# dacase/rnamotif

Measured on NVIDIA B200. Metric: strand-nt scanned per second (both strands), higher is better.
Workload: dtype u8

## Files before the change

rnamotif_b200/csrc/gm_kernel.cuh:

```cuda
#pragma once

#include <cuda_runtime.h>
#include <stdint.h>
#include "gm_search.cuh"
#include "gm_score.h"
#include "gm_twobit.h"
#include "gm_inflate.h"

namespace gm {


#define GM_REC_CACHE 30

#define PV (*L.P)

struct ScanArgs {
	DevParams par;
	const gm_plan_t *plan;
	const DevSearch *ds;
	const uint8_t *packed;
	int64_t total_nt;
	const int64_t *rec_off;
	int n_rec;
	int64_t g_begin, g_end;
// ... 42 lines not shown
			for (int k = 0; k < 4; k++) {
				uint32_t x = 0;
				for (int b = 0; b < 4; b++) {
					int64_t j = i + k * 4 + b;
					x |= (uint32_t)(j < n ? chars[j] : 0) << (8 * b);
				}
				w[k] = x;
			}
		}
		uint32_t out[2] = {0, 0};
		for (int k = 0; k < 16; k++) {
			unsigned ch = (w[k >> 2] >> (8 * (k & 3))) & 0xff;
			unsigned c = ch ? code_of_char(ch) : 0;
			out[k >> 3] |= c << (4 * (k & 7));
		}
		*reinterpret_cast<uint2 *>(packed + (i >> 1)) = make_uint2(out[0], out[1]);
	}
}

__device__ __forceinline__ int64_t last_le(const int64_t *__restrict__ a, int64_t lo, int64_t hi, int64_t x)
{
	while (lo < hi) {
		const int64_t mid = (lo + hi + 1) >> 1;
		if (a[mid] <= x)
			lo = mid;
		else
			hi = mid - 1;
	}
	return lo;
}

__device__ __forceinline__ int64_t first_ge2(const int64_t *__restrict__ a, int64_t lo, int64_t hi, int64_t x)
{
	while (lo < hi) {
		const int64_t mid = (lo + hi) >> 1;
		if (a[2 * mid] < x)
			lo = mid + 1;
		else
			hi = mid;
	}
	return lo;
}

__global__ void __launch_bounds__(256) gm_unpack2_kernel(const uint8_t *__restrict__ src,
	const int64_t *__restrict__ dna_off, const int64_t *__restrict__ rec_off, int n_rec,
	const int64_t *__restrict__ nblk, int64_t n_nblk, int64_t g0, int64_t n, uint8_t *__restrict__ packed)
{
	__shared__ int64_t br[4];
	const int64_t span = 256 * 16, end = g0 + n;
	for (int64_t b0 = g0 + (int64_t)blockIdx.x * span; b0 < end; b0 += (int64_t)gridDim.x * span) {
		const int64_t b1 = min(b0 + span, end);
		if (threadIdx.x == 0)
			br[0] = last_le(rec_off, 0, n_rec - 1, b0);
		else if (threadIdx.x == 1)
			br[1] = last_le(rec_off, 0, n_rec - 1, b1 - 1);
		else if (threadIdx.x == 2) {
			int64_t lo = 0, hi = n_nblk;
			while (lo < hi) {
				const int64_t mid = (lo + hi) >> 1;
				if (nblk[2 * mid + 1] <= b0)
					lo = mid + 1;
				else
					hi = mid;
			}
			br[2] = lo;
		} else if (threadIdx.x == 3)
			br[3] = first_ge2(nblk, 0, n_nblk, b1);
		__syncthreads();
		const int64_t r_lo = br[0], r_hi = br[1], k_lo = br[2], k_hi = br[3];
		const int64_t gg = b0 + (int64_t)threadIdx.x * 16;
		if (gg < b1) {
			const int64_t r = last_le(rec_off, r_lo, r_hi, gg);
			bool fast = gg + 16 <= rec_off[r + 1] && gg + 16 <= end;
			if (fast && k_lo < k_hi) {
				const int64_t k = first_ge2(nblk, k_lo, k_hi, gg + 16) - 1;
				fast = k < k_lo || nblk[2 * k + 1] <= gg;
			}
			uint32_t lo = 0, hi = 0;
			if (fast) {
				const int64_t q = gg - rec_off[r];
				const int phase = (int)(q & 3);
				const uint8_t *s = src + dna_off[r] + (q >> 2);
				const uint32_t be4 = ((uint32_t)s[0] << 24) | ((uint32_t)s[1] << 16) | ((uint32_t)s[2] << 8) | s[3];
				const uint32_t b4 = phase ? s[4] : 0;
				twobit_expand16(twobit_window(be4, b4, phase), lo, hi);
			} else {
				for (int j = 0; j < 16; j++) {
					const int64_t g = gg + j;
					if (g >= end)
						break;
					const int64_t rr = last_le(rec_off, r_lo, r_hi, g);
					const int64_t q = g - rec_off[rr];
					uint32_t code = twobit_code4((src[dna_off[rr] + (q >> 2)] >> (6 - 2 * (int)(q & 3))) & 3);
					if (k_lo < k_hi) {
						const int64_t k = first_ge2(nblk, k_lo, k_hi, g + 1) - 1;
						if (k >= k_lo && g < nblk[2 * k + 1])
							code = 15;
					}
					if (j < 8)
						lo |= code << (4 * j);
					else
						hi |= code << (4 * (j - 8));
				}
			}
			*reinterpret_cast<uint2 *>(packed + (gg >> 1)) = make_uint2(lo, hi);
		}
		__syncthreads();
	}
}

struct BgzfMember {
	uint64_t src;
	uint64_t dst;
	uint32_t len;
	uint32_t isize;
	uint32_t crc;
	uint32_t pad_;
};

__global__ void __launch_bounds__(32) gm_inflate_kernel(const uint8_t *__restrict__ gz, const BgzfMember *__restrict__ mem,
	int m0, int m1, uint8_t *__restrict__ text, uint8_t *__restrict__ status, unsigned int *__restrict__ first_bad)
{
	__shared__ uint32_t crc_tab[256];
	for (int i = threadIdx.x; i < 256; i += blockDim.x)
		crc_tab[i] = crc32_entry((uint32_t)i);
	__syncthreads();
	const int m = m0 + (int)(blockIdx.x * blockDim.x + threadIdx.x);
	if (m >= m1)
		return;
	const BgzfMember e = mem[m];
	uint32_t n_out;
	int st = inflate(gz + e.src, e.len, text + e.dst, e.isize, &n_out);
	if (st == GM_INF_OK && crc32(crc_tab, text + e.dst, e.isize) != e.crc)
		st = GM_INF_CRC;
	status[m] = (uint8_t)st;
	if (st != GM_INF_OK)
		atomicMin(first_bad, (unsigned int)m);
}


__device__ __forceinline__ uint32_t smem_u32(const void *p)
{
	return (uint32_t)__cvta_generic_to_shared(p);
}
__device__ __forceinline__ void mbar_init(uint64_t *bar, int count)
{
	asm volatile("mbarrier.init.shared::cta.b64 [%0], %1;" ::"r"(smem_u32(bar)), "r"(count));
	asm volatile("fence.mbarrier_init.release.cluster;" ::: "memory");
}
__device__ __forceinline__ void mbar_expect_tx(uint64_t *bar, uint32_t bytes)
{
	asm volatile("mbarrier.arrive.expect_tx.shared::cta.b64 _, [%0], %1;" ::"r"(smem_u32(bar)), "r"(bytes)
		: "memory");
}
__device__ __forceinline__ void tma_bulk_g2s(void *dst, const void *src, uint32_t bytes, uint64_t *bar)
{
	asm volatile(
		"cp.async.bulk.shared::cluster.global.mbarrier::complete_tx::bytes [%0], [%1], %2, [%3];" ::"r"(
			smem_u32(dst)),
		"l"(src), "r"(bytes), "r"(smem_u32(bar))
		: "memory");
}
__device__ __forceinline__ void mbar_wait(uint64_t *bar, uint32_t parity)
{
	asm volatile(
		"{\n"
		".reg .pred p;\n"
		"WAIT_%=:\n"
		"mbarrier.try_wait.parity.shared::cta.b64 p, [%0], %1;\n"
		"@p bra DONE_%=;\n"
		"bra WAIT_%=;\n"
		"DONE_%=:\n"
		"}\n" ::"r"(smem_u32(bar)),
		"r"(parity)
		: "memory");
}


__host__ __device__ inline size_t plan_smem_bytes(const DevParams &par)
{
	size_t n = 0;
	n += (sizeof(PlanView) + 15) & ~(size_t)15;
	n += (par.n_searches * sizeof(DevSearch) + 15) & ~(size_t)15;
	n += (par.n_descr * sizeof(gm_elem_t) + 15) & ~(size_t)15;
	n += (par.n_pairsets * sizeof(gm_pairset_t) + 15) & ~(size_t)15;
	n += (par.n_regex * sizeof(DevRegex) + 15) & ~(size_t)15;
	n += ((size_t)par.n_scopes * 4 + 15) & ~(size_t)15;
	n += ((size_t)par.n_lentab + 15) & ~(size_t)15;
	n += (par.n_sites * sizeof(gm_site_t) + 15) & ~(size_t)15;
	n += ((size_t)par.n_descr * 4 + 15) & ~(size_t)15;
	n += 2 * (((size_t)(par.n_descr + 1) * 4 + 15) & ~(size_t)15);
	return n;
}

struct StagedPlan {
	PlanView *pv;
	DevSearch *ds;
	const gm_pairset_t *ps;
	uint32_t *elmm;
	int *pmin, *pmax;
};

__device__ __forceinline__ void copy_words(void *dst, const void *src, int n_words, int tid, int nt)
{
	for (int i = tid; i < n_words; i += nt)
		reinterpret_cast<uint32_t *>(dst)[i] = reinterpret_cast<const uint32_t *>(src)[i];
}

__device__ __forceinline__ uint8_t *stage_plan(uint8_t *p, const ScanArgs &A, int tid, int nt, StagedPlan &sp)
{
	const DevParams &par = A.par;
	const gm_plan_t *pl = A.plan;
	PlanView *pv = reinterpret_cast<PlanView *>(p);         p += (sizeof(PlanView) + 15) & ~(size_t)15;
	DevSearch *ds = reinterpret_cast<DevSearch *>(p);       p += (par.n_searches * sizeof(DevSearch) + 15) & ~(size_t)15;
	gm_elem_t *el = reinterpret_cast<gm_elem_t *>(p);       p += (par.n_descr * sizeof(gm_elem_t) + 15) & ~(size_t)15;
	gm_pairset_t *ps = reinterpret_cast<gm_pairset_t *>(p); p += (par.n_pairsets * sizeof(gm_pairset_t) + 15) & ~(size_t)15;
	DevRegex *rx = reinterpret_cast<DevRegex *>(p);         p += (par.n_regex * sizeof(DevRegex) + 15) & ~(size_t)15;
	int32_t *sc = reinterpret_cast<int32_t *>(p);           p += ((size_t)par.n_scopes * 4 + 15) & ~(size_t)15;
	uint8_t *lt = p;                                        p += ((size_t)par.n_lentab + 15) & ~(size_t)15;
	gm_site_t *si = reinterpret_cast<gm_site_t *>(p);       p += (par.n_sites * sizeof(gm_site_t) + 15) & ~(size_t)15;
	uint32_t *elmm = reinterpret_cast<uint32_t *>(p);       p += ((size_t)par.n_descr * 4 + 15) & ~(size_t)15;
	int *pmin = reinterpret_cast<int *>(p);                 p += ((size_t)(par.n_descr + 1) * 4 + 15) & ~(size_t)15;
	int *pmax = reinterpret_cast<int *>(p);                 p += ((size_t)(par.n_descr + 1) * 4 + 15) & ~(size_t)15;
	for (int i = tid; i < (int)(sizeof(DevParams) / 4); i += nt)
		reinterpret_cast<uint32_t *>(&pv->par)[i] = reinterpret_cast<const uint32_t *>(&A.par)[i];
	copy_words(ds, A.ds, par.n_searches * (int)(sizeof(DevSearch) / 4), tid, nt);
	copy_words(el, pl->elems, par.n_descr * (int)(sizeof(gm_elem_t) / 4), tid, nt);
	copy_words(ps, pl->pairsets, par.n_pairsets * (int)(sizeof(gm_pairset_t) / 4), tid, nt);
	for (int r = 0; r < par.n_regex; r++)
		copy_words(rx + r, &pl->regex[r], (int)(sizeof(DevRegex) / 4), tid, nt);
	copy_words(sc, pl->scopes, par.n_scopes, tid, nt);
	copy_words(lt, pl->lentab, (par.n_lentab + 3) / 4, tid, nt);
	copy_words(si, pl->sites, par.n_sites * (int)(sizeof(gm_site_t) / 4), tid, nt);
	for (int i = tid; i < par.n_descr; i += nt)
		elmm[i] = pk16(pl->elems[i].minlen, pl->elems[i].maxlen);
	if (tid == 0) {
		int a = 0, b = 0;
		for (int i = 0; i <= par.n_descr; i++) {
			pmin[i] = a;
			pmax[i] = b;
			if (i < par.n_descr) {
				a += pl->elems[i].minlen;
				b += pl->elems[i].maxlen;
			}
		}
		pv->elems = el;
		pv->pairsets = ps;
		pv->regex = rx;
		pv->scopes = sc;
		pv->lentab = lt;
		pv->sites = si;
		pv->lctx = pl->lctx;
		pv->rctx = pl->rctx;
		pv->n_sites = par.n_sites;
		pv->n_pairsets = par.n_pairsets;
		pv->n_regex = par.n_regex;
		pv->pad_ = 0;
	}
	sp.pv = pv;
	sp.ds = ds;
	sp.ps = ps;
	sp.elmm = elmm;
	sp.pmin = pmin;
	sp.pmax = pmax;
	return p;
}


__device__ __noinline__ uint32_t el_word_lite(const Lane &L, int d)
{
	const int s = PV.par.elsrc[d];
	const int type = PV.elems[d].type;
	const int z = lo16(L_ZD(L, s));
	if (type == GM_SS)
		return pk16(z, lo16(L_FR(L, s, 0)) - z + 1);
	const int hl = hi16(L_FR(L, s, 3));
	if (type == GM_H5)
		return pk16(z, hl);
	return pk16(hi16(L_FR(L, s, 2)) - hl + 1, hl);
}
__device__ __forceinline__ int m_off(const Lane &L, int d) { return lo16(el_word(L, d, PV.par.lite != 0)); }
__device__ __forceinline__ int m_len(const Lane &L, int d) { return hi16(el_word(L, d, PV.par.lite != 0)); }

__device__ __noinline__ int wtype(const Lane &L, int p)
{
	for (int d = 0; d < L.ND; d++) {
		uint32_t w = el_word(L, d, PV.par.lite != 0);
		int off = lo16(w), len = hi16(w);
		if (len > 0 && p >= off && p < off + len)
			return PV.elems[d].type;
	}
	return -1;
}
__device__ __forceinline__ bool is_ss(const Lane &L, int p, bool undef_is_ss)
{
	int t = wtype(L, p);
	return t == GM_SS || (undef_is_ss && t < 0);
}

__device__ __noinline__ bool sink_strict(const Lane &L)
{
	for (int d = 0; d < L.ND; d++) {
		const gm_elem_t &e = PV.elems[d];
		if (!e.strict)
			continue;
		if (e.type == GM_H5) {
// ... 485 lines not shown
```

rnamotif_b200/csrc/gm_machine.cuh:

```cuda
#pragma once

#include "gm_kernel.cuh"
#include "gm_tilebits.h"

namespace gm {

enum {
	CL_IDLE = 0, CL_SPAN = 1, CL_WX = 2, CL_PK = 3, CL_TR = 4, CL_QU = 5
};
enum {
	PHX_IDLE = 0,
	PHX_ENTER = CL_SPAN * 8, PHX_SPAN, PHX_SS_RESUME, PHX_PH_RESUME, PHX_WC_RESUME,
	PHX_WX_BEGIN = CL_WX * 8, PHX_WX_RESUME, PHX_WX_FIRST, PHX_WX_EXT,
	PHX_PK_S5 = CL_PK * 8, PHX_PK_S3, PHX_PK_SD,
	PHX_TR_RESUME = CL_TR * 8, PHX_TR_S,
	PHX_QU_S1 = CL_QU * 8, PHX_QU_RESUME, PHX_QU_S2
};

#define PH_IDLE PHX_IDLE
#define PH_ENTER PHX_ENTER
#define PH_SPAN PHX_SPAN
#define PH_SS_RESUME PHX_SS_RESUME
#define PH_PH_RESUME PHX_PH_RESUME
#define PH_WC_RESUME PHX_WC_RESUME
#define PH_WX_BEGIN PHX_WX_BEGIN
#define PH_WX_RESUME PHX_WX_RESUME
#define PH_WX_FIRST PHX_WX_FIRST
#define PH_WX_EXT PHX_WX_EXT
#define PH_PK_S5 PHX_PK_S5
#define PH_PK_S3 PHX_PK_S3
#define PH_PK_SD PHX_PK_SD
#define PH_TR_RESUME PHX_TR_RESUME
#define PH_TR_S PHX_TR_S
#define PH_QU_S1 PHX_QU_S1
#define PH_QU_RESUME PHX_QU_RESUME
#define PH_QU_S2 PHX_QU_S2

#define GM_RETURN()                                  \
	do {                                             \
		if (s == 0)                                  \
			ph = PH_IDLE;                            \
		else {                                       \
			s--;                                     \
			ph = hi16(L_FR(L, s, 1));                \
		}                                            \
	} while (0)

#define FR1_LO(mpr, lbpr, chk) (((mpr) & 0xff) | ((lbpr) << 8) | ((chk) << 9))

#define GM_QCAP 128
#define GM_REFILL_MIN 16

struct WarpTile {
	uint64_t bar;
	int r_lo;
	int one_rec;
};

__device__ __forceinline__ uint8_t expand_code(unsigned c)
{
	unsigned b = c == 1 ? 0 : c == 2 ? 1 : c == 4 ? 2 : c == 8 ? 3 : 4;
	return (uint8_t)(c | (b << 4));
}
__device__ __forceinline__ uint8_t complement_byte(uint8_t v)
{
	unsigned b = v >> 4;
	if (b > 3)
		return (uint8_t)(15 | (4 << 4));
	unsigned nb = 3 - b;
	return (uint8_t)((1u << nb) | (nb << 4));
}

__device__ __forceinline__ uint64_t bits64(const uint32_t *set_, int q)
{
	const uint32_t *set = gm_sh(set_);
	const int w = q >> 5, sh = q & 31;
	const uint32_t a = set[w], b = set[w + 1], c = set[w + 2];
	const uint32_t lo = __funnelshift_r(a, b, sh);
	const uint32_t hi = __funnelshift_r(b, c, sh);
	return (uint64_t)lo | ((uint64_t)hi << 32);
}

struct PairBits {
	const uint32_t *base;
	int nwb;
	int n_dups;
};

__device__ __forceinline__ uint64_t wc_mask_body(const PairBits &pb, const uint8_t *sq, int strand, int sqbase,
	int dupi, int flt, int z, int lo, int n)
{
	const uint64_t ones = n >= 64 ? ~0ull : ((1ull << n) - 1);
	const int req = flt & 0xff, budget = (flt >> 8) & 0xff, first_must = (flt >> 16) & 1;
	if (dupi < 0 || req == 0)
		return ones;
	const uint32_t *sets = pb.base + ((size_t)(strand * pb.n_dups + dupi) * 4) * pb.nwb;
	if (budget == 0 && first_must) {
		uint64_t a = ones;
		for (int k = 0; k < req; k++) {
			const int x = bcode_of(sq[z + k]);
			if (x >= 4)
				return 0;
			a &= bits64(sets + x * pb.nwb, sqbase + lo - k);
		}
		return a;
	}
	uint64_t a0 = ones, a1 = ones, a2 = ones;
	for (int k = 0; k < req; k++) {
		const int x = bcode_of(sq[z + k]);
		uint64_t m = 0;
		if (x < 4)
			m = bits64(sets + x * pb.nwb, sqbase + lo - k);
		if (k == 0 && first_must) {
			a0 = a1 = a2 = m;
		} else if (k == 0 && budget == 0) {
		} else {
			a2 = (a2 & m) | a1;
			a1 = (a1 & m) | a0;
			a0 &= m;
		}
	}
	return (budget == 0 ? a0 : budget == 1 ? a1 : a2) & ones;
}

__device__ __noinline__ uint64_t wc_mask(const PairBits &pb, const uint8_t *sq, int strand, int sqbase,
	int dupi, int flt, int z, int lo, int n)
{
	return wc_mask_body(pb, sq, strand, sqbase, dupi, flt, z, lo, n);
}

template <int REQ, typename Fin>
__device__ __forceinline__ uint32_t sieve_word_r(const PairBits &pb, int strand, int dupi, int flt, int w, int Dlo, int Dhi, Fin fin)
{
	constexpr int NS_ = REQ > 0 ? REQ : 8;
	const int req = REQ > 0 ? REQ : (flt & 0xff);
	const int budget = (flt >> 8) & 0xff, first_must = (flt >> 16) & 1;
	const int nwb = pb.nwb;
	const uint32_t *P = gm_sh(pb.base) + ((size_t)(strand * pb.n_dups + dupi) * 4) * nwb;
	const uint32_t *I = gm_sh(pb.base) + ((size_t)(strand * pb.n_dups) * 4) * nwb;
	uint32_t Bl[4], Bh[4];
#pragma unroll
	for (int x = 0; x < 4; x++) {
		Bl[x] = I[x * nwb + w];
		Bh[x] = I[x * nwb + w + 1];
	}
	uint32_t res = 0;
	const int Dmin = Dlo - 2 * (req - 1);
	for (int par = 0; par < 2; par++) {
		uint32_t a0[NS_], a1[NS_];
#pragma unroll
		for (int u = 0; u < NS_; u++)
			a0[u] = a1[u] = ~0u;
		for (int d = Dmin + par; d <= Dhi; d += 2) {
			const int ww = min(w + (d >> 5), nwb - 3), sh = d & 31;
			uint32_t Ml = 0, Mh = 0;
#pragma unroll
			for (int x = 0; x < 4; x++) {
				const uint32_t c0 = P[x * nwb + ww], c1 = P[x * nwb + ww + 1], c2 = P[x * nwb + ww + 2];
				Ml |= Bl[x] & __funnelshift_r(c0, c1, sh);
				Mh |= Bh[x] & __funnelshift_r(c1, c2, sh);
			}
#pragma unroll
			for (int k = NS_ - 1; k >= 1; k--) {
				if (REQ > 0 || k < req) {
					const uint32_t t = __funnelshift_r(Ml, Mh, k);
					a1[k] = (a1[k] & t) | a0[k];
					a0[k] &= t;
				}
			}
			uint32_t f;
			if (first_must)
				f = (budget ? a1[0] : a0[0]) & Ml;
			else if (budget == 0)
				f = a0[0];
			else
				f = (a1[0] & Ml) | a0[0];
			if (d >= Dlo)
				res |= fin(d, f);
#pragma unroll
			for (int u = 0; u < NS_ - 1; u++) {
				a0[u] = a0[u + 1];
				a1[u] = a1[u + 1];
			}
			a0[NS_ - 1] = a1[NS_ - 1] = ~0u;
		}
	}
	return res;
}

template <typename Fin>
__device__ __forceinline__ uint32_t sieve_word(const PairBits &pb, int strand, int dupi, int flt, int w, int Dlo, int Dhi, Fin fin)
{
	return sieve_word_r<0>(pb, strand, dupi, flt, w, Dlo, Dhi, fin);
}
template <typename Fin>
__device__ __forceinline__ uint32_t sieve_word_main(const PairBits &pb, int strand, int dupi, int flt, int w, int Dlo, int Dhi, Fin fin)
{
	switch (flt & 0xff) {
	case 3: return sieve_word_r<3>(pb, strand, dupi, flt, w, Dlo, Dhi, fin);
	case 4: return sieve_word_r<4>(pb, strand, dupi, flt, w, Dlo, Dhi, fin);
	case 5: return sieve_word_r<5>(pb, strand, dupi, flt, w, Dlo, Dhi, fin);
	case 6: return sieve_word_r<6>(pb, strand, dupi, flt, w, Dlo, Dhi, fin);
	case 7: return sieve_word_r<7>(pb, strand, dupi, flt, w, Dlo, Dhi, fin);
	}
	return sieve_word_r<0>(pb, strand, dupi, flt, w, Dlo, Dhi, fin);
}

__device__ __forceinline__ uint32_t bits32(const uint32_t *set_, int q)
{
	const uint32_t *set = gm_sh(set_);
	return __funnelshift_r(set[q >> 5], set[(q >> 5) + 1], q & 31);
}

__device__ __noinline__ uint64_t wc_mask_rev(const PairBits &pb, const uint8_t *sq, int strand, int sqbase,
	int dupi_t, int flt, int e, int zlo, int n)
{
	const uint64_t ones = n >= 64 ? ~0ull : ((1ull << n) - 1);
	const int req = flt & 0xff, budget = (flt >> 8) & 0xff, first_must = (flt >> 16) & 1;
	if (dupi_t < 0 || req == 0)
		return ones;
	const uint32_t *sets = pb.base + ((size_t)(strand * pb.n_dups + dupi_t) * 4) * pb.nwb;
	uint64_t a0 = ones, a1 = ones, a2 = ones;
	for (int k = 0; k < req; k++) {
		const int y = bcode_of(sq[e - k]);
		uint64_t m = 0;
		if (y < 4)
			m = bits64(sets + y * pb.nwb, sqbase + zlo + k);
		if (k == 0 && first_must) {
			a0 = a1 = a2 = m;
		} else if (k == 0 && budget == 0) {
		} else {
			a2 = (a2 & m) | a1;
			a1 = (a1 & m) | a0;
			a0 &= m;
		}
	}
	return (budget == 0 ? a0 : budget == 1 ? a1 : a2) & ones;
}

__device__ __forceinline__ bool tail_feasible(const PairBits &pb, const uint8_t *sq, int strand, int sqbase,
	const DevSearch &S, const DevSearch &T, int s5, int s3, int hl)
{
	const int e = s3 - hl - S.lk_off;
	int zhi = e - T.dlo;
	const int zlo = max(e - T.dhi, s5 + hl);
	for (; zhi >= zlo; zhi -= 64) {
		const int l0 = max(zlo, zhi - 63);
		if (wc_mask_rev(pb, sq, strand, sqbase, T.dupi_t, T.flt, e, l0, zhi - l0 + 1) != 0)
			return true;
	}
	return false;
}

#define GM_LOOK_FWD(any, T, zt, bound)                                   \
	do {                                                                 \
		int f_ = min((bound), (zt) + (T).dhi);                           \
		const int l_ = (zt) + (T).dlo;                                   \
		(any) = false;                                                   \
		for (; f_ >= l_ && !(any); f_ -= 64) {                           \
			const int l0_ = max(l_, f_ - 63);                            \
			(any) = GM_MASK((T), (zt), l0_, f_ - l0_ + 1) != 0;          \
		}                                                                \
	} while (0)

__device__ __noinline__ bool probes_ok(const Lane &L, const DevSearch &S, int s5, int s3, int hl, int wend)
{
	for (int i = 0; i < S.n_probe; i++) {
		const unsigned pr = S.probe[i];
		const int anchor = pr & 3, off = (pr >> 2) & 1023, len = (pr >> 12) & 255;
		const int rxi = (pr >> 20) & 31, mm = (pr >> 25) & 15;
		const int pos = anchor == 0 ? s5 + hl + off : anchor == 1 ? s3 + 1 + off : s3 - hl + 1 - off - len;
		if (pos < 0 || pos + len - 1 > wend)
			return false;
		const DevRegex &rx = PV.regex[rxi];
		int n_mm;
		if (mm > 0 ? !rx_match_mm(rx, L.sq + pos, len, mm, &n_mm) : !rx_match(rx, L.sq + pos, len))
			return false;
	}
	return true;
}

template <int MODE, bool FULL, int PF>
__device__ __forceinline__ void gm_search_body(const ScanArgs &A)
{
	constexpr bool SIEVE = PF >= 2;
	const bool LIT = PF == 1 || (SIEVE && A.par.lit_present != 0);
	extern __shared__ __align__(16) uint8_t smem_raw[];
	const int tid = threadIdx.x, nt = blockDim.x;
	const int lane = tid & 31, warp = tid >> 5;
	const int NS = A.par.n_searches, ND = A.par.n_descr;
	const int W = A.par.w_winsize, H = A.par.halo, TILE = A.par.tile;
	const int Lbytes = (TILE + 2 * H + 31) & ~31;
	const int stage_bytes = ((Lbytes >> 1) + 32 + 15) & ~15;
	const int nwb = ((Lbytes + 31) >> 5) + 4;
	const int n_dups = A.par.n_dups;
	const int NBUF = MODE == 0 ? 2 : 1;

	const int nwarps = nt >> 5;
	const size_t pb_bytes = (((size_t)2 * n_dups * 4 * nwb * 4) + 15) & ~(size_t)15;
	const size_t lit_bytes = LIT ? (((size_t)2 * nwb * 4) + 15) & ~(size_t)15 : 0;
	const size_t buf_bytes = 2 * (size_t)Lbytes + pb_bytes + (GM_REC_CACHE + 2) * 8 + lit_bytes;
	const bool CHAIN = SIEVE && A.par.chain > 0;
	const size_t warp_bytes = 16 + (size_t)stage_bytes + NBUF * buf_bytes + GM_QCAP * 2 + (SIEVE ? ((6 * (size_t)nwb * 4 + 15) & ~(size_t)15) : 0) +
		(CHAIN ? ((6 * (size_t)nwb * 4 + 15) & ~(size_t)15) : 0);
	StagedPlan sp;
	uint8_t *p = stage_plan(smem_raw, A, tid, nt, sp);
	DevSearch *sm_ds = sp.ds;
	uint64_t *sm_litB = reinterpret_cast<uint64_t *>(p);       p += LIT ? 16 * 8 : 0;
	uint8_t *wp = p + (size_t)warp * warp_bytes;               p += (size_t)nwarps * warp_bytes;
	uint32_t *sm_state = reinterpret_cast<uint32_t *>(p);
	WarpTile *sm = reinterpret_cast<WarpTile *>(wp);           wp += 16;
	uint8_t *sm_stage = wp;                                    wp += stage_bytes;
	uint8_t *bufs = wp;                                        wp += NBUF * buf_bytes;
	uint16_t *myq = reinterpret_cast<uint16_t *>(wp);
	uint32_t *sv_E = reinterpret_cast<uint32_t *>(myq + GM_QCAP);
	uint32_t *sv_K = sv_E + 2 * nwb;
	uint32_t *sv_K2 = sv_K + 2 * nwb;
	uint32_t *ch_F = reinterpret_cast<uint32_t *>(reinterpret_cast<uint8_t *>(sv_E) + (SIEVE ? ((6 * (size_t)nwb * 4 + 15) & ~(size_t)15) : 0));
	uint32_t *ch_OK = ch_F + 4 * nwb;
	const uint32_t *ch_F0 = ch_F;
	const bool deep = SIEVE && A.par.pf_deep != 0;
	constexpr bool TWO = MODE == 1 && PF == 3;
	const bool ST2 = TWO || (MODE == 1 && SIEVE && A.par.sv_helix != 0 && A.par.pf_search >= 0 &&
		A.ds[max(A.par.pf_search, 0)].n_probe > 0);
	const int sv_nws = ((TILE - 1) >> 5) + 2;
	const int sv_npass = (A.strands * sv_nws + 31) >> 5;

	if (LIT && tid < 16)
		sm_litB[tid] = A.plan->regex[A.par.lit_rx].B[tid];
	if (lane == 0)
		mbar_init(&sm->bar, 1);

	Lane L;
	L.P = sp.pv;
	L.st = sm_state + tid;
	L.nt = nt;
	L.ds = sm_ds;
	L.ps = sp.ps;
	L.NS = NS;
	L.ND = ND;
	L.el_base = NS + A.par.frame_words;
	L.sq = bufs;
	L.szero = L.slen = L.comp = 0;
	L.rec = 0;
	L.seq = 0;
	if (MODE == 0) {
		for (int d = 0; FULL && d < ND; d++) {
			unmark(L, d);
			set_cnt(L, d, GM_UNDEF, GM_UNDEF);
		}
	}
	__syncthreads();

	uint32_t parity = 0;
	unsigned long long my_starts = 0;
	unsigned my_entries = 0;

	int cur = NBUF - 1;
	bool have_tile = false, no_more_tiles = false;
	int64_t gA = 0, gB = 0, lo = 0;
	uint8_t *sm_fwd = bufs, *sm_rc = bufs;
	int64_t *sm_rec = reinterpret_cast<int64_t *>(bufs);
	PairBits pb;
	pb.base = reinterpret_cast<uint32_t *>(bufs);
	pb.nwb = nwb;
	pb.n_dups = n_dups;
	uint32_t *sm_lit = reinterpret_cast<uint32_t *>(bufs);
	bool one_rec = false;
	int r_lo = 0;
	int64_t rec0_off = 0;
	int rec0_len = 0;
	int work_next = 0;
	const int n_work = A.strands * TILE;
	const int refill_min = A.par.refill_min;

	int sqbase = 0, strand = 0, mybuf = 0;
	PairBits mypb = pb;

	auto load_tile = [&](int b, int64_t t) {
		uint8_t *bp = bufs + (size_t)b * buf_bytes;
		sm_fwd = bp;
		sm_rc = bp + Lbytes;
		pb.base = reinterpret_cast<uint32_t *>(bp + 2 * (size_t)Lbytes);
		sm_rec = reinterpret_cast<int64_t *>(bp + 2 * (size_t)Lbytes + pb_bytes);
		sm_lit = reinterpret_cast<uint32_t *>(bp + 2 * (size_t)Lbytes + pb_bytes + (GM_REC_CACHE + 2) * 8);
		gA = A.g_begin + t * (int64_t)TILE;
		gB = min(gA + (int64_t)TILE, A.g_end);
		lo = gA - H;
		const int64_t lo_c = max(lo, (int64_t)0);
		const int64_t hi_c = min(lo + Lbytes, A.total_nt);
		const int64_t bs = (lo_c >> 1) & ~(int64_t)15;
		const uint32_t nbytes = (uint32_t)((((hi_c + 1) >> 1) - bs + 15) & ~(int64_t)15);
		if (lane == 0) {
			mbar_expect_tx(&sm->bar, nbytes);
			tma_bulk_g2s(sm_stage, A.packed + bs, nbytes, &sm->bar);
			int a = 0, bb = A.n_rec;
			while (bb - a > 1) {
				int m = (a + bb) >> 1;
				if (A.rec_off[m] <= gA)
					a = m;
				else
					bb = m;
			}
			sm->r_lo = a;
			sm->one_rec = A.rec_off[a + 1] >= gB;
		}
		__syncwarp();
		r_lo = sm->r_lo;
		one_rec = sm->one_rec != 0;
		for (int i = lane; i <= GM_REC_CACHE; i += 32) {
			int r = r_lo + i;
			sm_rec[i] = r <= A.n_rec ? A.rec_off[r] : (int64_t)1 << 62;
		}
		mbar_wait(&sm->bar, parity);
		parity ^= 1;
		uint32_t *pbw = const_cast<uint32_t *>(pb.base);
		const int nw = Lbytes >> 5;
		{
			const uint32_t *stw = reinterpret_cast<const uint32_t *>(sm_stage);
			const int n_stw = stage_bytes >> 2;
			const int base_q = (int)(lo - 2 * bs);
			const int sh = (base_q & 7) * 4;
			const bool edge = lo < 0 || lo + Lbytes > A.total_nt;
			const unsigned sel1 = (lane & 1) ? 0x3715u : 0x6240u, sel2 = (lane & 2) ? 0x3276u : 0x5410u;
			for (int i0 = lane * 8; i0 < ((Lbytes + 255) & ~255); i0 += 256) {
				const int wq = (base_q + i0) >> 3;
				const uint32_t w0 = stw[min(max(wq, 0), n_stw - 1)], w1 = stw[min(max(wq + 1, 0), n_stw - 1)];
				uint32_t x = __funnelshift_r(w0, w1, sh);
				if (edge) {
					const int64_t g0 = lo + i0;
					const int klo = (int)min((int64_t)8, max((int64_t)0, -g0));
					const int khi = (int)min((int64_t)8, max((int64_t)0, A.total_nt - g0));
					const uint32_t m_hi = khi >= 8 ? ~0u : ((1u << (4 * khi)) - 1u);
					const uint32_t m_lo = klo >= 8 ? 0u : (~0u << (4 * klo));
					x &= m_hi & m_lo;
				}
				uint32_t f0, f1, r0, r1, bits;
				expand8(x, f0, f1, r0, r1, bits);
				uint32_t o = __shfl_xor_sync(0xffffffffu, bits, 1);
				bits = __byte_perm(bits, o, sel1);
				o = __shfl_xor_sync(0xffffffffu, bits, 2);
				bits = __byte_perm(bits, o, sel2);
				if (i0 < Lbytes) {
					*reinterpret_cast<uint2 *>(sm_fwd + i0) = make_uint2(f0, f1);
					*reinterpret_cast<uint2 *>(sm_rc + Lbytes - 8 - i0) = make_uint2(r0, r1);
					pbw[(size_t)(lane & 3) * nwb + (i0 >> 5)] = bits;
				}
			}
		}
		if (lane < 4 * (nwb - nw))
			pbw[(size_t)(lane / (nwb - nw)) * nwb + nw + lane % (nwb - nw)] = 0;
		__syncwarp();
		for (int x = 0; x < 4; x++)
			for (int w = lane; w < nwb; w += 32)
				pbw[((size_t)(n_dups * 4) + x) * nwb + w] = w < nw ? __brev(pbw[(size_t)(3 - x) * nwb + nw - 1 - w]) : 0u;
		__syncwarp();
		for (int sd = 0; sd < 2 * n_dups; sd++) {
			const int st = sd >= n_dups, dd = st ? sd - n_dups : sd;
			if (dd == 0)
				continue;
			const unsigned dup = A.par.dups[dd];
			const uint32_t *bs_ = pbw + (size_t)(st * n_dups) * 4 * nwb;
			uint32_t *out = pbw + (size_t)(st * n_dups + dd) * 4 * nwb;
			for (int x = 0; x < 4; x++) {
				const unsigned row = dup >> (x * 5);
				for (int w = lane; w < nwb; w += 32) {
					uint32_t acc = 0;
#pragma unroll
					for (int y = 0; y < 4; y++)
						if ((row >> y) & 1u)
							acc |= bs_[(size_t)y * nwb + w];
					out[(size_t)x * nwb + w] = acc;
				}
			}
		}
		if (LIT) {
			const int len = A.par.lit_len, l_mm = A.par.lit_mm;
			const uint64_t dot = PV.regex[A.par.lit_rx].dot;
			const uint64_t sel0 = sm_litB[1], sel1 = sm_litB[2], sel2 = sm_litB[4], sel3 = sm_litB[8];
			for (int idx = lane; idx < 2 * nwb; idx += 32) {
				const int st = idx >= nwb, w = idx - st * nwb;
				const uint32_t *Bs = pbw + (size_t)(st * n_dups) * 4 * nwb;
				uint32_t a0 = ~0u, a1 = ~0u, a2 = ~0u;
				for (int k = 0; k < len; k++) {
					if ((dot >> k) & 1)
						continue;
					const int q = min((w << 5) + k, Lbytes);
					const uint32_t b0 = bits32(Bs, q), b1 = bits32(Bs + nwb, q), b2 = bits32(Bs + 2 * nwb, q),
						b3 = bits32(Bs + 3 * nwb, q);
					const uint32_t m = ~(b0 | b1 | b2 | b3) | (((sel0 >> k) & 1) ? b0 : 0u) | (((sel1 >> k) & 1) ? b1 : 0u) |
						(((sel2 >> k) & 1) ? b2 : 0u) | (((sel3 >> k) & 1) ? b3 : 0u);
					a2 = (a2 & m) | a1;
					a1 = (a1 & m) | a0;
					a0 &= m;
				}
				sm_lit[idx] = l_mm == 0 ? a0 : l_mm == 1 ? a1 : l_mm == 2 ? a2 : ~0u;
			}
		}
		__syncwarp();
		rec0_off = sm_rec[0];
		rec0_len = (int)(sm_rec[1] - sm_rec[0]);
		work_next = 0;
		cur = b;
		have_tile = true;
	};

	auto next_tile = [&]() -> int64_t {
		unsigned long long t_ = 0;
		if (lane == 0)
			t_ = atomicAdd(A.tile_counter, 1ull);
		const int64_t t = (int64_t)__shfl_sync(0xffffffffu, t_, 0);
		return t < A.n_tiles ? t : -1;
	};

	auto locate = [&](int q, int &comp, int &idx, uint32_t &rec, int &slen, int &szero) -> bool {
		if (q >= n_work)
			return false;
		comp = q >= TILE;
		const int64_t g = gA + (comp ? q - TILE : q);
		if (g >= gB)
			return false;
		int64_t off;
		if (one_rec) {
			off = rec0_off;
			slen = rec0_len;
			rec = (uint32_t)r_lo;
		} else if (g < sm_rec[GM_REC_CACHE]) {
			int a = 0, b = GM_REC_CACHE;
			while (b - a > 1) {
				int m = (a + b) >> 1;
				if (sm_rec[m] <= g)
					a = m;
				else
					b = m;
			}
			off = sm_rec[a];
			slen = (int)(sm_rec[a + 1] - off);
			rec = (uint32_t)(a + r_lo);
		} else {
			int a = r_lo, b = A.n_rec;
			while (b - a > 1) {
				int m = (a + b) >> 1;
				if (A.rec_off[m] <= g)
					a = m;
				else
					b = m;
			}
			off = A.rec_off[a];
			slen = (int)(A.rec_off[a + 1] - off);
			rec = (uint32_t)a;
		}
		const int pos = (int)(g - off);
		szero = comp ? slen - 1 - pos : pos;
		idx = (int)(g - lo);
		return slen - szero >= A.par.dminlen;
	};

	auto prefilter = [&](int q, uint64_t &v0, int &have_v0) -> bool {
		int comp, idx, slen, szero;
		uint32_t rec;
		v0 = 0;
		have_v0 = 0;
		bool pass = locate(q, comp, idx, rec, slen, szero);
		if (!pass)
			return false;
		my_starts++;
		const DevSearch &S0 = sm_ds[0];
		const uint8_t *sq = comp ? sm_rc + (Lbytes - 1 - idx) : sm_fwd + idx;
		const int base = comp ? Lbytes - 1 - idx : idx;
		const int dl = min(W, slen - szero) - 1;
		if (LIT) {
			const int l = A.par.lit_lmin;
			int h = min(A.par.lit_lmax, dl + 1 - A.par.lit_len);
			bool any = false;
			const uint32_t *set = sm_lit + comp * nwb;
			for (; h >= l && !any; h -= 64) {
				const int l0 = max(l, h - 63), n = h - l0 + 1;
				const uint64_t ones = n >= 64 ? ~0ull : ((1ull << n) - 1);
				any = (bits64(set, base + l0) & ones) != 0;
			}
			if (!any)
				return false;
		}
		if (A.par.pf_search >= 0) {
			const DevSearch &SP = sm_ds[A.par.pf_search];
			const int pz = A.par.pf_z;
			const int fsd = min(dl, pz + SP.dhi), lsd = pz + SP.dlo;
			bool any = false;
			for (int hi = fsd; hi >= lsd && !any; hi -= 64) {
				const int l0 = max(lsd, hi - 63);
				const uint64_t v = wc_mask(pb, sq, comp, base, SP.dupi, SP.flt, pz, l0, hi - l0 + 1);
				any = v != 0;
				if (hi == fsd && l0 == lsd && SP.kind != K_PK && A.par.pf_search == 0) {
					v0 = v;
					have_v0 = 1;
				}
			}
			pass = any;
		}
		if (pass && S0.rx5 >= 0 && S0.mm5 == 0 && !PV.regex[S0.rx5].eol) {
			pass = rx_match(PV.regex[S0.rx5], sq, min(S0.maxlen, dl + 1)) != 0;
		}
		return pass;
	};

	auto accept = [&](int q) -> bool {
		int comp, idx, slen, szero;
		uint32_t rec;
		if (!locate(q, comp, idx, rec, slen, szero))
			return false;
		const DevSearch &S0 = sm_ds[0];
		if (S0.rx5 >= 0 && S0.mm5 == 0 && !PV.regex[S0.rx5].eol) {
			const uint8_t *sq = comp ? sm_rc + (Lbytes - 1 - idx) : sm_fwd + idx;
			const int dl = min(W, slen - szero) - 1;
			return rx_match(PV.regex[S0.rx5], sq, min(S0.maxlen, dl + 1)) != 0;
		}
		return true;
	};

	auto accept2 = [&](int q) -> bool {
		int comp, idx, slen, szero;
		uint32_t rec;
		if (!locate(q, comp, idx, rec, slen, szero))
			return false;
		const DevSearch &S0 = sm_ds[0];
		const DevSearch &SP = sm_ds[A.par.pf_search];
		const uint8_t *sq = comp ? sm_rc + (Lbytes - 1 - idx) : sm_fwd + idx;
		const int base = comp ? Lbytes - 1 - idx : idx;
		const int dl = min(W, slen - szero) - 1;
		if (S0.rx5 >= 0 && S0.mm5 == 0 && !PV.regex[S0.rx5].eol &&
		    !rx_match(PV.regex[S0.rx5], sq, min(S0.maxlen, dl + 1)))
			return false;
		const int pz = A.par.pf_z;
		const int lsd = pz + SP.dlo;
		const uint32_t *K = sv_K + comp * nwb;
		const bool use_k = deep && SP.kid_t >= 0;
		for (int hi = min(dl, pz + SP.dhi); hi >= lsd; hi -= 64) {
			const int l0 = max(lsd, hi - 63);
			uint64_t v = wc_mask(pb, sq, comp, base, SP.dupi, SP.flt, pz, l0, hi - l0 + 1);
			while (v) {
				const int s3 = l0 + __ffsll((long long)v) - 1;
				v &= v - 1;
				for (int hl = SP.minlen; hl <= SP.maxlen; hl++) {
					const int kp = base + pz + hl + SP.kid_off;
					if (use_k && !((K[kp >> 5] >> (kp & 31)) & 1u))
						continue;
					if (SP.lk_t >= 0 && !tail_feasible(pb, sq, comp, base, SP, sm_ds[SP.lk_t], pz, s3, hl))
						continue;
					if (SP.n_probe) {
						Lane Lq = L;
						Lq.sq = sq;
						if (!probes_ok(Lq, SP, pz, s3, hl, dl))
							continue;
					}
					return true;
				}
			}
		}
		return false;
	};

	auto chain_build = [&]() {
		const int nw = Lbytes >> 5;
		uint32_t *Fa = ch_F, *Fb = ch_F + 2 * nwb;
		for (int i = lane; i < 2 * nwb; i += 32)
			Fa[i] = ~0u;
		__syncwarp();
		const uint32_t *pbw = pb.base;
		for (int c = 0; c < A.par.chain; c++) {
			const unsigned w0 = A.par.chain_w0[c], w1 = A.par.chain_w1[c];
			const int mn = w0 & 4095, mx = (w0 >> 12) & 4095, cm = (w0 >> 24) & 15;
			const bool both = (w0 >> 28) & 1, con = (w0 >> 29) & 1;
			if (con) {
				for (int i = lane; i < 2 * nwb; i += 32) {
					const int st = i >= nwb, w = i - st * nwb;
					const uint32_t *Bs = pbw + (size_t)(st * n_dups) * 4 * nwb;
					ch_OK[i] = ((cm & 1) ? Bs[w] : 0u) | ((cm & 2) ? Bs[nwb + w] : 0u) | ((cm & 4) ? Bs[2 * nwb + w] : 0u) |
						((cm & 8) ? Bs[3 * nwb + w] : 0u);
				}
				__syncwarp();
			}
			for (int i = lane; i < 2 * nwb; i += 32) {
				const int st = i >= nwb, w = i - st * nwb;
				uint32_t out = ~0u;
				if (w < nw && st < A.strands) {
					const uint32_t *Fn = Fa + st * nwb;
					const int q0 = w << 5;
					out = 0;
					if (!con) {
						for (int len = mn; len <= mx && out != ~0u; len++)
							out |= bits32(Fn, min(q0 + len, Lbytes));
					} else {
						const uint32_t *OK = ch_OK + st * nwb;
						uint32_t a0 = ~0u, a1 = ~0u, a2 = ~0u;
						const uint32_t ok0 = OK[w];
						for (int k = 0; k < mx; k++) {
							const uint32_t m = bits32(OK, min(q0 + k, Lbytes));
							a2 = (a2 & m) | a1;
							a1 = (a1 & m) | a0;
							a0 &= m;
							const int hl = k + 1;
							if (hl >= mn) {
								const int b = (w1 >> (2 * (hl - mn))) & 3;
								uint32_t okh = b == 0 ? a0 : b == 1 ? a1 : b == 2 ? a2 : ~0u;
								if (both && b != 3)
									okh &= ok0 & m;
								out |= okh & bits32(Fn, min(q0 + hl, Lbytes));
							}
						}
					}
				}
				Fb[i] = out;
			}
			__syncwarp();
			uint32_t *t_ = Fa;
			Fa = Fb;
			Fb = t_;
		}
		ch_F0 = Fa;
	};

	auto sieve_aux = [&]() {
		const DevSearch &SP = sm_ds[A.par.pf_search];
		const int nw = Lbytes >> 5;
		for (int i = lane; i < 2 * nwb; i += 32) {
			sv_E[i] = 0;
			sv_K[i] = 0;
			sv_K2[i] = 0;
		}
		__syncwarp();
		const int nv = (int)(gB - gA);
		for (int st = 0; st < A.strands; st++) {
			const int zlo = (st ? Lbytes - H - nv : H) + A.par.pf_z, zhi = zlo + nv - 1;
			if (SP.lk_t >= 0 && !TWO) {
				const DevSearch &T = sm_ds[SP.lk_t];
				const int lo_ = max(zlo + SP.dlo - SP.maxlen - SP.lk_off - T.dhi, 0);
				const int hi_ = min(zhi + SP.dhi - SP.minlen - SP.lk_off - T.dlo, Lbytes - 1);
				uint32_t *E = sv_E + st * nwb;
				for (int w = (lo_ >> 5) + lane; w <= (hi_ >> 5) && w < nw; w += 32)
					sieve_word_main(pb, st, T.dupi, T.flt, w, T.dlo, T.dhi,
						[&](int d, uint32_t f) -> uint32_t {
							const int q = (w << 5) + d, sh = q & 31;
							if (f != 0) {
								if ((q >> 5) < nwb)
									atomicOr(E + (q >> 5), f << sh);
								if (sh && (q >> 5) + 1 < nwb)
									atomicOr(E + (q >> 5) + 1, f >> (32 - sh));
							}
							return 0u;
						});
			}
			if (SP.kid_t >= 0) {
				const DevSearch &T = sm_ds[SP.kid_t];
				const int lo_ = zlo + SP.minlen + SP.kid_off;
				const int hi_ = min(zhi + SP.maxlen + SP.kid_off + 31, Lbytes - 1);
				const bool has_k2 = A.par.pf_deep == 2;
				const uint32_t *K2 = sv_K2 + st * nwb;
				if (has_k2) {
					const DevSearch &T2 = sm_ds[T.sib_t];
					const int lo2 = (lo_ & ~31) + T.dlo + 1 + T.sib_off;
					const int hi2 = min((hi_ | 31) + T.dhi + 1 + T.sib_off + 31, Lbytes - 1);
					for (int w = (lo2 >> 5) + lane; w <= (hi2 >> 5) && w < nw; w += 32)
						sv_K2[st * nwb + w] = sieve_word_main(pb, st, T2.dupi, T2.flt, w, T2.dlo, T2.dhi,
							[](int, uint32_t f) -> uint32_t { return f; });
					__syncwarp();
				}
				const int k2off = T.sib_off + 1;
				for (int w = (lo_ >> 5) + lane; w <= (hi_ >> 5) && w < nw; w += 32)
					sv_K[st * nwb + w] = sieve_word_main(pb, st, T.dupi, T.flt, w, T.dlo, T.dhi,
						[&](int d, uint32_t f) -> uint32_t {
							return has_k2 ? f & bits32(K2, min((w << 5) + d + k2off, Lbytes)) : f;
						});
			}
		}
		__syncwarp();
	};
	auto sieve_pass = [&](int pass, int &strand_, int &w_) -> uint32_t {
		const DevSearch &SP = sm_ds[max(A.par.pf_search, 0)];
		const int pz = A.par.pf_z;
		const int nv = (int)(gB - gA);
		const int it = pass * 32 + lane;
		uint32_t word = 0;
		strand_ = it / sv_nws;
		w_ = 0;
		if (strand_ < A.strands) {
			const int zlo = (strand_ ? Lbytes - H - nv : H) + pz, zhi = zlo + nv - 1;
			w_ = (zlo >> 5) + it % sv_nws;
			if (w_ <= (zhi >> 5)) {
				const int nhl = deep ? SP.maxlen - SP.minlen + 1 : 1;
				const uint32_t *E = sv_E + strand_ * nwb, *K = sv_K + strand_ * nwb;
				uint32_t kh[4];
#pragma unroll
				for (int j = 0; j < 4; j++)
					kh[j] = j < nhl ? (deep && SP.kid_t >= 0 ? bits32(K, (w_ << 5) + SP.minlen + j + SP.kid_off) : ~0u) : 0u;
				const int e0 = (w_ << 5) - SP.minlen - SP.lk_off - (nhl - 1);
				const bool has_lk = deep && SP.lk_t >= 0;
				word = !A.par.sv_helix ? ~0u : TWO ? (kh[0] | kh[1] | kh[2] | kh[3]) :
					sieve_word_main(pb, strand_, SP.dupi, SP.flt, w_, SP.dlo, SP.dhi,
					[&](int d, uint32_t f) -> uint32_t {
						if (!has_lk)
							return f & (kh[0] | kh[1] | kh[2] | kh[3]);
						const int q = max(e0 + d, 0);
						const uint32_t x0 = E[q >> 5], x1 = E[(q >> 5) + 1], x2 = E[(q >> 5) + 2];
						const uint32_t lo_ = __funnelshift_r(x0, x1, q & 31), hi_ = __funnelshift_r(x1, x2, q & 31);
						uint32_t la = 0;
#pragma unroll
						for (int j = 0; j < 4; j++)
// ... 92 lines not shown
							q = sieve_pop(word, st_, w_);
							pass = accept(q);
						}
						wl_append(pass, q, 0, 0);
					}
				}
				if (qtail != qhead) {
					const bool mine = lane < qtail - qhead;
					const int q2 = mine ? myq[(qhead + lane) & (GM_QCAP - 1)] : 0;
					wl_append(mine && accept2(q2), q2, 0, 0);
				}
			} else {
				for (;;) {
					const int chunk = work_next;
					work_next += 32;
					if (chunk >= n_work)
						break;
					const int q = chunk + lane;
					uint64_t v0;
					int have_v0;
					const bool pass = prefilter(q, v0, have_v0);
					wl_append(pass, q, v0, have_v0);
				}
			}
			__syncwarp();
		}
	} else {
		int s = 0, ph = PH_IDLE;
		int qhead = 0, qtail = 0;
		constexpr bool sieve = SIEVE;
		int sv_pass = 0, sv_strand = 0, sv_w = 0;
		uint32_t sw = 0;

		for (;;) {
			const unsigned idle = __ballot_sync(0xffffffffu, ph == PH_IDLE);
			if (__popc(idle) >= refill_min || (idle && no_more_tiles)) {
				const int want = __popc(idle);
				while (qtail - qhead < want) {
					const unsigned sv_left = sieve ? __ballot_sync(0xffffffffu, sw != 0) : 0u;
					if (!have_tile || (sieve ? (sv_left == 0 && sv_pass >= sv_npass) : work_next >= n_work)) {
						if (no_more_tiles)
							break;
						if (qtail != qhead)
							break;
						const int nb = (cur + 1) % NBUF;
						if (__ballot_sync(0xffffffffu, ph != PH_IDLE && mybuf == nb))
							break;
						const int64_t t = next_tile();
						if (t < 0) {
							no_more_tiles = true;
							have_tile = false;
							break;
						}
						load_tile(nb, t);
						sv_pass = 0;
						sw = 0;
						if (CHAIN)
							chain_build();
						if (deep)
							sieve_aux();
						continue;
					}
					if (sieve) {
						if (sv_left == 0) {
							sw = sieve_pass(sv_pass, sv_strand, sv_w);
							sv_pass++;
							continue;
						}
						int q = 0;
						bool pass = false;
						if (sw != 0) {
							q = sieve_pop(sw, sv_strand, sv_w);
							pass = accept(q);
						}
						const unsigned pm = __ballot_sync(0xffffffffu, pass);
						if (pass)
							myq[(qtail + __popc(pm & ((1u << lane) - 1))) & (GM_QCAP - 1)] = (uint16_t)q;
						qtail += __popc(pm);
						__syncwarp();
						continue;
					}
					const int chunk = work_next;
					work_next += 32;
					const int q = chunk + lane;
					uint64_t v0;
					int have_v0;
					const bool pass = prefilter(q, v0, have_v0);
					const unsigned pm = __ballot_sync(0xffffffffu, pass);
					if (pass)
						myq[(qtail + __popc(pm & ((1u << lane) - 1))) & (GM_QCAP - 1)] = (uint16_t)q;
					qtail += __popc(pm);
					__syncwarp();
				}
				const int avail = qtail - qhead;
				const int rank = __popc(idle & ((1u << lane) - 1));
				if (ph == PH_IDLE && rank < avail) {
					const int q = myq[(qhead + rank) & (GM_QCAP - 1)];
					int comp, idx, slen, szero;
					uint32_t rec;
					locate(q, comp, idx, rec, slen, szero);
					L.rec = rec;
					L.slen = slen;
					L.szero = szero;
					L.comp = comp;
					L.seq = 0;
					strand = comp;
					sqbase = comp ? Lbytes - 1 - idx : idx;
					L.sq = (comp ? sm_rc : sm_fwd) + sqbase;
					mybuf = cur;
					mypb = pb;
					L_ZD(L, 0) = pk16(0, min(W, slen - szero) - 1);
					s = 0;
					ph = PH_ENTER;
					my_entries++;
				}
				qhead += min(avail, want);
				__syncwarp();
				if (no_more_tiles && qtail == qhead && __all_sync(0xffffffffu, ph == PH_IDLE))
					break;
			}

#define GM_MASK(S, z, clo, n)                                                                          \
	(FULL ? wc_mask_body(mypb, L.sq, strand, sqbase, (S).dupi, (S).flt, (z), (clo), (n))               \
	      : wc_mask(mypb, L.sq, strand, sqbase, (S).dupi, (S).flt, (z), (clo), (n)))
#define GM_TAIL(S, T, s5, s3, hl) tail_feasible(mypb, L.sq, strand, sqbase, (S), (T), (s5), (s3), (hl))
#define GM_BBITS(x, p) bits64(mypb.base + ((size_t)(strand * mypb.n_dups) * 4 + (x)) * mypb.nwb, sqbase + (p))
#define GM_FULL FULL
#include "gm_machine_body.inc"
#undef GM_FULL
#undef GM_TAIL
#undef GM_BBITS
#undef GM_MASK
		}
	}

	for (int o = 16; o > 0; o >>= 1)
		my_starts += __shfl_down_sync(0xffffffffu, my_starts, o);
	if (lane == 0 && my_starts)
		atomicAdd(A.start_count, my_starts);
	my_entries = __reduce_add_sync(0xffffffffu, my_entries);
	if (lane == 0 && my_entries)
		atomicAdd(A.start_count + 3, (unsigned long long)my_entries);
}

template <int MODE, bool FULL, int PF>
__global__ void gm_search_kernel(const ScanArgs A)
{
	gm_search_body<MODE, FULL, PF>(A);
}
template <int PF>
__global__ void __launch_bounds__(256, 2) gm_filter_kernel(const ScanArgs A)
{
	gm_search_body<1, false, PF>(A);
}

template <bool FULL>
__global__ void gm_dfs_kernel(const ScanArgs A)
{
	extern __shared__ __align__(16) uint8_t smem_raw[];
	const int tid = threadIdx.x, nt = blockDim.x;
	const int lane = tid & 31;
	const int NS = A.par.n_searches, ND = A.par.n_descr;
	const int W = A.par.w_winsize;
	const int Lc = A.par.halo - W;
	const int wstride = A.par.win_stride;
	const int Wtot = W + 2 * Lc;

	StagedPlan sp;
	uint8_t *p = stage_plan(smem_raw, A, tid, nt, sp);
	DevSearch *sm_ds = sp.ds;
	uint8_t *sm_win = p;                                       p += (size_t)nt * wstride;
	uint32_t *sm_bits = reinterpret_cast<uint32_t *>(p);       p += (size_t)nt * A.par.win_bits * 4;
	uint32_t *sm_state = reinterpret_cast<uint32_t *>(p);

	Lane L;
	L.P = sp.pv;
	L.st = sm_state + tid;
	L.nt = nt;
	L.ds = sm_ds;
	L.ps = sp.ps;
	L.NS = NS;
	L.ND = ND;
	L.el_base = NS + A.par.frame_words;
	uint8_t *mywin = sm_win + (size_t)tid * wstride;
	L.sq = mywin + Lc;
	PairBits mypb;
	mypb.base = sm_bits + (size_t)tid * A.par.win_bits;
	mypb.nwb = ((Wtot + 31) >> 5) + 3;
	mypb.n_dups = A.par.n_dups;
	L.szero = L.slen = L.comp = 0;
	L.rec = 0;
	L.seq = 0;
	for (int d = 0; FULL && d < ND; d++) {
		unmark(L, d);
		set_cnt(L, d, GM_UNDEF, GM_UNDEF);
	}
	__syncthreads();

	const unsigned long long wl_n = min(*A.wl_count, A.wl_cap);
	int s = 0, ph = PH_IDLE;
	bool exhausted = false;
	const int nwl = mypb.nwb;
	const unsigned long long n_warps = (unsigned long long)gridDim.x * (blockDim.x >> 5);
	const int per = (int)max(1ull, min(32ull, (wl_n + n_warps - 1) / n_warps));
	const int rmin = min(A.par.dfs_refill, per);
	const unsigned long long gwarp = (unsigned long long)blockIdx.x * (blockDim.x >> 5) + (tid >> 5);
	int taken = 0;

	for (;;) {
		const unsigned idle = __ballot_sync(0xffffffffu, ph == PH_IDLE);
		if (!exhausted && (__popc(idle) >= rmin || idle == 0xffffffffu)) {
			const int n = min(__popc(idle), per);
			const int rank = __popc(idle & ((1u << lane) - 1));
			unsigned long long mine;
			if (per < 32) {
				mine = (unsigned long long)(taken + rank) * n_warps + gwarp;
				taken += n;
				if ((unsigned long long)taken * n_warps + gwarp >= wl_n)
					exhausted = true;
			} else {
				unsigned long long base = 0;
				if (lane == 0)
					base = atomicAdd(A.wl_head, (unsigned long long)n);
				base = __shfl_sync(0xffffffffu, base, 0);
				if (base + n >= wl_n)
					exhausted = true;
				mine = base + rank;
			}
			if (ph == PH_IDLE && rank < n && mine < wl_n) {
				const uint4 *e = reinterpret_cast<const uint4 *>(A.wl + mine * GM_WL_WORDS);
				const uint4 e0 = e[0], e1v = e[1];
				L.rec = e0.z;
				L.slen = (int)e0.w;
				L.szero = (int)e1v.x;
				L.comp = (int)(e0.y >> 31);
				L.seq = 0;
				const int64_t roff = A.rec_off[L.rec];
				const int slen = L.slen, comp = L.comp, c00 = L.szero - Lc;
				uint32_t *mb = const_cast<uint32_t *>(mypb.base);
				const uint32_t *pw = reinterpret_cast<const uint32_t *>(A.packed);
				const int64_t wmax = (A.total_nt >> 3) + 1;
				uint32_t *win32 = reinterpret_cast<uint32_t *>(mywin);
				for (int w = 0; w < nwl; w++) {
					uint32_t b0 = 0, b1 = 0, b2 = 0, b3 = 0;
					const int i0 = w << 5;
					if (!FULL) {
#pragma unroll
					for (int g = 0; g < 4; g++) {
						const int t0 = i0 + 8 * g;
						if (t0 < Wtot) {
							const int c0 = c00 + t0;
							const int jlo = max(0, -c0), jhi = min(min(8, slen - c0), Wtot - t0);
							uint32_t x = 0;
							if (jhi > jlo) {
								const int64_t f0 = comp ? roff + (slen - 1 - (c0 + 7)) : roff + c0;
								const int64_t wi = f0 >> 3;
								const int sh = (int)(f0 & 7) * 4;
								x = __funnelshift_r(pw[max((int64_t)0, min(wi, wmax))], pw[max((int64_t)0, min(wi + 1, wmax))], sh);
								if (jlo > 0 || jhi < 8) {
									const int nlo = comp ? 8 - jhi : jlo, nhi = comp ? 8 - jlo : jhi;
									x &= (nhi >= 8 ? ~0u : ((1u << (4 * nhi)) - 1u)) & (~0u << (4 * nlo));
								}
							}
							uint32_t f0_, f1_, r0_, r1_, bits;
							expand8(x, f0_, f1_, r0_, r1_, bits);
							if (comp) {
								f0_ = r0_;
								f1_ = r1_;
								bits = __brev(bits);
								if (jlo > 0 || jhi < 8) {
									for (int jj = 0; jj < 8; jj++)
										if (jj < jlo || jj >= jhi) {
											uint32_t &wd = jj < 4 ? f0_ : f1_;
											wd = (wd & ~(0xffu << (8 * (jj & 3)))) | (0x40u << (8 * (jj & 3)));
										}
								}
							}
							win32[t0 >> 2] = f0_;
							if (t0 + 4 < Wtot)
								win32[(t0 >> 2) + 1] = f1_;
							b0 |= (bits & 0xffu) << (8 * g);
							b1 |= ((bits >> 8) & 0xffu) << (8 * g);
							b2 |= ((bits >> 16) & 0xffu) << (8 * g);
							b3 |= (bits >> 24) << (8 * g);
						}
					}
					} else {
					for (int t = 0; t < 32 && i0 + t < Wtot; t++) {
						const int c = c00 + i0 + t;
						uint8_t v = (uint8_t)(4 << 4);
						if (c >= 0 && c < slen) {
							const int64_t gf = roff + (comp ? slen - 1 - c : c);
							const unsigned byte = A.packed[gf >> 1];
							v = expand_code((byte >> ((gf & 1) * 4)) & 15);
							if (comp)
								v = complement_byte(v);
						}
						mywin[i0 + t] = v;
						const int bc = bcode_of(v);
						b0 |= (uint32_t)(bc == 0) << t;
						b1 |= (uint32_t)(bc == 1) << t;
						b2 |= (uint32_t)(bc == 2) << t;
						b3 |= (uint32_t)(bc == 3) << t;
					}
					}
					mb[0 * nwl + w] = b0;
// ... 36 lines not shown
```

rnamotif_b200/csrc/gm_machine_body.inc:

```
			const int cls = ph >> 3;
			const unsigned peers = __match_any_sync(0xffffffffu, cls);
			const int vote = cls == CL_IDLE ? 0 : ((__popc(peers) << 4) | cls);
			const int run_cls = __reduce_max_sync(0xffffffffu, vote) & 15;
			int pend = 0, pc0 = -1, pc1 = -1, pc2 = -1, pc3 = -1;
			if (cls == run_cls) {

			int wc_stage = 0;
			switch (run_cls) {
			case CL_SPAN: {
				if (ph == PH_WC_RESUME) {
					if (GM_FULL) {
						unmark(L, sm_ds[s].d);
						unmark(L, sm_ds[s].d3);
					}
					wc_stage = 1;
				} else if (ph == PH_SS_RESUME) {
					if (GM_FULL)
						unmark(L, sm_ds[s].d);
				} else if (ph == PH_PH_RESUME) {
					unmark(L, sm_ds[s].d);
					unmark(L, sm_ds[s].d3);
				} else if (ph == PH_ENTER) {
				const DevSearch &S = sm_ds[s];
				const uint32_t zd = L_ZD(L, s);
// ... 19 lines not shown
					const int d0 = sc[0], dn = sc[e.n_scopes - 1];
					const uint32_t r4 = pk_range(L, sp, S, S.d3 + 1, dn);
					L_FR(L, s, 9) = pk_range(L, sp, S, d0, S.d - 1);
					L_FR(L, s, 10) = pk_range(L, sp, S, S.d, dn);
					L_FR(L, s, 11) = pk16(lo16(pk_range(L, sp, S, S.d + 1, S.d3 - 1)), lo16(r4));
					L_FR(L, s, 12) = pk16(hi16(r4), 0);
					{
						const uint32_t w9 = L_FR(L, s, 9);
						if (lo16(w9) == hi16(w9) && S.dhi - S.dlo < 64) {
							const int s5 = z + lo16(w9);
							const int n = min(S.dhi, dl - s5) - S.dlo + 1;
							const uint64_t V = n > 0 ? GM_MASK(S, s5, s5 + S.dlo, n) : 0ull;
							if (V == 0) {
								GM_RETURN();
								break;
							}
							L_FR(L, s, 16) = (uint32_t)V;
							L_FR(L, s, 17) = (uint32_t)(V >> 32);
							L_FR(L, s, 12) = pk16(lo16(L_FR(L, s, 12)), 1);
						}
					}
					if (S.d == sc[1]) {
						const int d3_h1 = PV.elems[sc[0]].mates[0];
						L_FR(L, s, 13) = pk_range(L, sp, S, S.d + 1, d3_h1 - 1);
						L_FR(L, s, 14) = pk_range(L, sp, S, d3_h1 + 1, S.d3 - 1);
						L_FR(L, s, 15) = pk16(m_off(L, d3_h1) - 1, m_off(L, d3_h1) + m_len(L, d3_h1));
					}
				}
				}
				if (GM_FULL && sm_ds[s].kind == K_PK) {
					ph = PH_PK_SD;
					break;
				}
				ph = PH_SPAN;
				const DevSearch &S = sm_ds[s];
				const uint32_t zd = L_ZD(L, s);
				const int z = lo16(zd), dl = hi16(zd);
				const uint32_t w0 = L_FR(L, s, 0);
				int sd = lo16(w0) - 1;
				const int lsd = hi16(w0);

				if (S.kind == K_SS) {
					for (;; sd--) {
						if (sd < lsd) {
							GM_RETURN();
							break;
						}
						const int len = sd - z + 1;
						int mm = 0;
						if (S.rx5 >= 0 && !chk_seq5(L, S, z, len, mm))
							continue;
						if (GM_FULL) {
							set_cnt(L, S.d, 0, mm);
							mark(L, S.d, z, len);
						}
						if (S.next_s >= 0)
							L_ZD(L, S.next_s) = pk16(sd + 1, dl);
						L_FR(L, s, 0) = pk16(sd, lsd);
						L_FR(L, s, 1) = pk16(mm, PH_SS_RESUME);
						if (S.last) {
							int ctx_[4];
							if (!sink_pass(L, ctx_)) {
								if (GM_FULL)
									unmark(L, S.d);
								continue;
							}
							pend = 1;
							pc0 = ctx_[0]; pc1 = ctx_[1]; pc2 = ctx_[2]; pc3 = ctx_[3];
							ph = PH_SS_RESUME;
							break;
						}
						s++;
						ph = PH_ENTER;
						break;
					}
					break;
				}

				if (S.kind == K_WC) {
					const int s5 = z;
					int top = sd, clo = hi16(L_FR(L, s, 4));
					uint64_t v = (uint64_t)L_FR(L, s, 5) | ((uint64_t)L_FR(L, s, 6) << 32);
					int s3 = 0, s3lim = 0, hl = 0, mpr = 0, lbpr = 1;
					if (wc_stage) {
						const uint32_t w3 = L_FR(L, s, 3);
						const int f1 = lo16(L_FR(L, s, 1));
						s3 = hi16(L_FR(L, s, 2));
						s3lim = lo16(w3);
						hl = hi16(w3);
						mpr = f1 & 0xff;
						lbpr = (f1 >> 8) & 1;
					}
					for (;;) {
						bool cand = false;
						if (!wc_stage) {
							while (v == 0) {
								if (top < lsd)
									break;
								clo = max(lsd, top - 63);
								v = GM_MASK(S, z, clo, top - clo + 1);
								top = clo - 1;
							}
							if (v == 0) {
								GM_RETURN();
								break;
							}
							const int j = 63 - __clzll((long long)v);
							v &= ~(1ull << j);
							s3 = clo + j;
							if (S.sib_t >= 0) {
								const DevSearch &T = sm_ds[S.sib_t];
								bool any;
								GM_LOOK_FWD(any, T, s3 + 1 + S.sib_off, dl);
								if (!any) {
									L_FR(L, s, 0) = pk16(top + 1, lsd);
									L_FR(L, s, 4) = pk16(0, clo);
									L_FR(L, s, 5) = (uint32_t)v;
									L_FR(L, s, 6) = (uint32_t)(v >> 32);
									break;
								}
							}
							int t3 = s3 - z + 1;
							t3 = (t3 - S.minilen) / 2;
							t3 = min(t3, S.maxlen);
							s3lim = s3 - t3 + 1;
							hl = 0; mpr = 0; lbpr = 1;
							wc_stage = 1;
							if (GM_FULL && S.hmm) {
								set_cnt(L, S.d, 0, 0);
								set_cnt(L, S.d3, 0, 0);
							}
							cand = S.minlen == 0 && s3 - s5 + 1 <= S.maxilen;
						}
						if (!cand) {
							const bool more = (GM_FULL && S.hmm) ? wx_next_mm(L, S, s5, s3, s3lim, &hl, &mpr, &lbpr)
							                                     : wx_next(L, S, s5, s3, s3lim, hl, mpr, lbpr);
							if (!more) {
								L_FR(L, s, 0) = pk16(top + 1, lsd);
								L_FR(L, s, 4) = pk16(0, clo);
								L_FR(L, s, 5) = (uint32_t)v;
								L_FR(L, s, 6) = (uint32_t)(v >> 32);
								break;
							}
							if (s3 - s5 - 2 * hl + 1 > S.maxilen)
								continue;
							if (S.lk_t >= 0 && !GM_TAIL(S, sm_ds[S.lk_t], s5, s3, hl))
								continue;
							if (S.kid_t >= 0) {
								bool any;
								GM_LOOK_FWD(any, sm_ds[S.kid_t], s5 + hl + S.kid_off, s3 - hl);
								if (!any)
									continue;
							}
							if (S.n_probe && !probes_ok(L, S, s5, s3, hl, hi16(L_ZD(L, 0))))
								continue;
						}
						L_FR(L, s, 0) = pk16(top + 1, lsd);
						L_FR(L, s, 1) = pk16(FR1_LO(mpr, lbpr, 0), PH_WC_RESUME);
						L_FR(L, s, 2) = pk16(s5, s3);
						L_FR(L, s, 3) = pk16(s3lim, hl);
						L_FR(L, s, 4) = pk16(0, clo);
						L_FR(L, s, 5) = (uint32_t)v;
						L_FR(L, s, 6) = (uint32_t)(v >> 32);
						if (GM_FULL) {
							if (S.hmm) {
								wx_finish_mm(L, S, s5, s3, s3lim, hl, mpr, lbpr);
								set_mpr(L, S.d, mpr);
								set_mpr(L, S.d3, mpr);
							} else {
								set_cnt(L, S.d, mpr, 0);
								set_cnt(L, S.d3, mpr, 0);
							}
							mark(L, S.d, s5, hl);
							mark(L, S.d3, s3 - hl + 1, hl);
						}
						if (S.next_s >= 0)
							L_ZD(L, S.next_s) = pk16(s3 + 1, dl);
						L_ZD(L, s + 1) = pk16(s5 + hl, s3 - hl);
						s++;
						ph = PH_ENTER;
						break;
					}
					break;
				}
				if (S.kind == K_QU) {
					uint64_t v = (uint64_t)L_FR(L, s, 5) | ((uint64_t)L_FR(L, s, 6) << 32);
					int clo = hi16(L_FR(L, s, 4));
					int top = sd;
					while (v == 0) {
						if (top < lsd)
							break;
						clo = max(lsd, top - 63);
						v = GM_MASK(S, z, clo, top - clo + 1);
						top = clo - 1;
					}
					if (v == 0) {
						L_FR(L, s, 0) = pk16(top + 1, lsd);
						GM_RETURN();
						break;
					}
					const int j = 63 - __clzll((long long)v);
					v &= ~(1ull << j);
					sd = clo + j;
					L_FR(L, s, 5) = (uint32_t)v;
					L_FR(L, s, 6) = (uint32_t)(v >> 32);
					L_FR(L, s, 4) = pk16(0, clo);
					L_FR(L, s, 0) = pk16(top + 1, lsd);
					if (S.sib_t >= 0) {
						bool any;
						GM_LOOK_FWD(any, sm_ds[S.sib_t], sd + 1 + S.sib_off, dl);
						if (!any)
							break;
					}
				} else {
					if (sd < lsd) {
						GM_RETURN();
						break;
					}
					L_FR(L, s, 0) = pk16(sd, lsd);
				}
				if (S.next_s >= 0)
					L_ZD(L, S.next_s) = pk16(sd + 1, dl);

				if (!GM_FULL)
					break;
				switch (S.kind) {
				case K_QU: {
					const gm_elem_t &e = PV.elems[S.d];
					set_cnt(L, S.d, 0, 0);
					set_cnt(L, S.d3, 0, 0);
					set_cnt(L, e.mates[0], 0, 0);
					set_cnt(L, e.mates[1], 0, 0);
					const int i_minl = S.minilen + PV.elems[e.mates[0]].minilen +
						PV.elems[e.mates[1]].minilen + 2 * S.minlen;
					int t3 = sd - z + 1;
					t3 = (t3 - i_minl) / 2;
					t3 = min(t3, S.maxlen);
					const int s3lim = sd - t3 + 1;
					L_FR(L, s, 2) = pk16(z, sd);
					L_FR(L, s, 3) = pk16(s3lim, 0);
					ph = S.minlen == 0 ? PH_WX_BEGIN : PH_WX_FIRST;
					break;
				}
				case K_PH: {
					set_cnt(L, S.d, 0, 0);
					set_cnt(L, S.d3, 0, 0);
					const int slen = sd - z + 1;
					int s5hi = min((slen - S.minilen) / 2, S.maxlen);
					s5hi = z + s5hi - 1;
					int ilen = slen - 2 * S.minlen;
					ilen = min(ilen, S.maxilen);
					int s5lo = slen - ilen;
					if (s5lo & 1)
						s5lo++;
					s5lo = min(s5lo / 2, S.maxlen);
					s5lo = z + s5lo - 1;
					int hlen, n_mpr;
					if (!match_phlx(L, S, S.d3, z, sd, s5hi, s5lo, &hlen, &n_mpr))
						break;
					if (sd - z - 2 * hlen + 1 > S.maxilen)
						break;
					set_mpr(L, S.d, n_mpr);
					set_mpr(L, S.d3, n_mpr);
					mark(L, S.d, z, hlen);
					mark(L, S.d3, sd - hlen + 1, hlen);
					L_ZD(L, s + 1) = pk16(z + hlen, sd - hlen);
					L_FR(L, s, 1) = pk16(0, PH_PH_RESUME);
					s++;
					ph = PH_ENTER;
					break;
				}
				case K_TR: {
					const gm_elem_t &e = PV.elems[S.d];
					const int dd1 = e.mates[0], dd2 = e.mates[1];
					const gm_elem_t &e1 = PV.elems[dd1];
					set_cnt(L, S.d, 0, 0);
					set_cnt(L, dd1, 0, 0);
					set_cnt(L, dd2, 0, 0);
					const int slen = sd - z + 1;
					int s5hi = min((slen - S.minilen - e1.minilen) / 2, S.maxlen);
					s5hi = z + s5hi - 1;
					int i_len = slen - 2 * S.minlen;
					i_len = min(i_len, S.maxilen + S.minlen + e1.maxilen);
					int s5lo = slen - i_len;
					if (s5lo & 1)
						s5lo++;
					s5lo = min(s5lo / 2, S.maxlen);
					s5lo = z + s5lo - 1;
					int hlen, n_mpr;
					if (!match_phlx(L, S, dd2, z, sd, s5hi, s5lo, &hlen, &n_mpr))
						break;
					if (sd - z - 2 * hlen + 1 > S.maxilen + e1.maxilen + hlen)
						break;
					mark(L, S.d, z, hlen);
					mark(L, dd2, sd - hlen + 1, hlen);
					L_FR(L, s, 2) = pk16(z, sd);
					L_FR(L, s, 4) = pk16(sd - e1.minilen - hlen + 1, hlen);
					ph = PH_TR_S;
					break;
				}
				}
				break;
			}

			case CL_WX: {
				if (!GM_FULL)
					break;
				if (ph == PH_WX_BEGIN) {
				const DevSearch &S = sm_ds[s];
				const uint32_t w2 = L_FR(L, s, 2);
				const int s5 = lo16(w2), s3 = hi16(w2);
				L_FR(L, s, 1) = pk16(FR1_LO(0, 1, 0), PH_WX_RESUME);
				if (S.kind == K_QU) {
					mark(L, S.d, s5, 0);
					mark(L, S.d3, s3 + 1, 0);
					L_FR(L, s, 7) = pk16(s5 + S.minilen - 1, 0);
					L_FR(L, s, 8) = 0x40000000u;
					ph = PH_QU_S1;
				} else
					ph = PH_WX_FIRST;
				break;
				}
				if (ph == PH_WX_RESUME) {
					unmark(L, sm_ds[s].d);
					unmark(L, sm_ds[s].d3);
					ph = hi16(L_FR(L, s, 3)) == 0 ? PH_WX_FIRST : PH_WX_EXT;
				}
				{
				const DevSearch &S = sm_ds[s];
				const uint32_t w2 = L_FR(L, s, 2), w3 = L_FR(L, s, 3);
				const int s5 = lo16(w2), s3 = hi16(w2), s3lim = lo16(w3);
				int hl, mpr, lbpr, chk;
				if (ph == PH_WX_FIRST) {
					if (paired(S.duplex, L.sq[s5], L.sq[s3])) {
						hl = 1; mpr = 0; lbpr = 1;
					} else if (!(S.ends & GM_5PAIRED)) {
						hl = 1; mpr = 1; lbpr = 0;
					} else {
						ph = S.kind == K_PK ? PH_PK_S3 : PH_SPAN;
						break;
					}
					chk = 1;
				} else {
					const int f1 = lo16(L_FR(L, s, 1));
					hl = hi16(w3);
					mpr = f1 & 0xff;
					lbpr = (f1 >> 8) & 1;
					chk = (f1 >> 9) & 1;
				}
				int found = 0;
				for (;;) {
					if (chk) {
						chk = 0;
						if (hl >= S.minlen &&
						    !(!lbpr && (S.ends & GM_3PAIRED)) &&
						    !(S.pfrac && mpr > PV.lentab[S.lentab + hl]) &&
						    !(S.rx5 >= 0 && !chk_seq_el(L, S.d, s5, hl)) &&
						    !(S.rx3 >= 0 && !chk_seq_el(L, S.d3, s3 - hl + 1, hl))) {
							if (S.kind == K_PK) {
								const int i_minl = hi16(L_FR(L, s, 5));
								if ((s3 - s5 + 1) - 2 * hl < i_minl) {
									found = -1;
									break;
								}
								found = 1;
								const gm_elem_t &e = PV.elems[S.d];
								const int *sc = &PV.scopes[e.scopes];
								if (S.d == sc[1]) {
									const uint32_t w13 = L_FR(L, s, 13), w14 = L_FR(L, s, 14), w15 = L_FR(L, s, 15);
									const int iL_minl = lo16(w13), iL_maxl = hi16(w13);
									const int iR_minl = lo16(w14), iR_maxl = hi16(w14);
									const int iL_last = lo16(w15), iR_last = hi16(w15);
									const int iL = iL_last - (s5 + hl - 1);
									const int iR = (s3 - hl + 1) - iR_last;
									if (iL < iL_minl || iL > iL_maxl || iR < iR_minl || iR > iR_maxl)
										found = 0;
								}
							} else
								found = 1;
							if (found > 0 && S.lk_t >= 0 && !GM_TAIL(S, sm_ds[S.lk_t], s5, s3, hl))
								found = 0;
							if (found > 0 && S.kid_t >= 0) {
								bool any;
								GM_LOOK_FWD(any, sm_ds[S.kid_t], s5 + hl + S.kid_off, (S.nest & 1) ? s3 - hl : hi16(L_ZD(L, 0)));
								if (!any)
									found = 0;
							}
							if (found > 0 && S.n_probe && !probes_ok(L, S, s5, s3, hl, hi16(L_ZD(L, 0))))
								found = 0;
							if (found)
								break;
						}
					}
					if (s3 - hl + 1 < s3lim || hl >= S.maxlen) {
						found = -1;
						break;
					}
					if (paired(S.duplex, L.sq[s5 + hl], L.sq[s3 - hl]))
						lbpr = 1;
					else {
						if (++mpr > S.mplim) {
							found = -1;
							break;
						}
						lbpr = 0;
					}
					hl++;
					chk = 1;
				}
				if (found < 0) {
					ph = S.kind == K_PK ? PH_PK_S3 : PH_SPAN;
					break;
				}
				if (S.hmm)
					wx_finish_mm(L, S, s5, s3, s3lim, hl, mpr, lbpr);
				L_FR(L, s, 3) = pk16(s3lim, hl);
				L_FR(L, s, 1) = pk16(FR1_LO(mpr, lbpr, 0), PH_WX_RESUME);
				mark(L, S.d, s5, hl);
				mark(L, S.d3, s3 - hl + 1, hl);
				if (S.kind == K_PK) {
					set_mpr(L, S.d, mpr);
					set_mpr(L, S.d3, mpr);
					upd_pksearches(L, S.d, s5, s3, hl);
					s++;
					ph = PH_ENTER;
				} else {
					L_FR(L, s, 7) = pk16(s5 + hl + S.minilen - 1, 0);
					L_FR(L, s, 8) = 0x40000000u;
					ph = PH_QU_S1;
				}
				break;
			}

			}

			case CL_PK: {
				if (!GM_FULL)
					break;
				const DevSearch &S = sm_ds[s];
				const gm_elem_t &e = PV.elems[S.d];
				for (int it = 0; it < 8; it++) {
					if (ph == PH_PK_SD && hi16(L_FR(L, s, 12)) != 0) {
						const uint32_t zd = L_ZD(L, s);
						const int z = lo16(zd), dl = hi16(zd);
						const uint32_t w0 = L_FR(L, s, 0);
						int sd = lo16(w0) - 1;
						const int lsd = hi16(w0);
						const uint32_t w9 = L_FR(L, s, 9), w10 = L_FR(L, s, 10), w11 = L_FR(L, s, 11);
						const int p_maxl = hi16(w9), r_minl = lo16(w10), r_maxl = hi16(w10);
						const int i_minl = lo16(w11), s_minl = hi16(w11), s_maxl = lo16(L_FR(L, s, 12));
						const int g_minl = 2 * S.minlen + i_minl;
						const int s5 = z + lo16(w9);
						const uint64_t V = (uint64_t)L_FR(L, s, 16) | ((uint64_t)L_FR(L, s, 17) << 32);
						uint64_t vsel = 0;
						int l_s3 = 0;
						for (; sd >= lsd; sd--) {
							const int slen = sd - z + 1;
							if (p_maxl + r_maxl < slen || s5 > z + min(p_maxl, slen - r_minl))
								continue;
							const int slen5 = sd - s5 + 1;
							if (g_minl + s_minl > slen5)
								continue;
							int f_s3 = min(sd - s_minl, s5 + S.dhi);
							l_s3 = max(sd - min(slen5 - g_minl, s_maxl), s5 + S.dlo);
							if (e.scope == 1) {
								const uint32_t w14 = L_FR(L, s, 14);
								const int iR_last = hi16(L_FR(L, s, 15));
								f_s3 = min(f_s3, iR_last + hi16(w14) + S.maxlen - 1);
								l_s3 = max(l_s3, iR_last + lo16(w14) + S.minlen - 1);
							}
							const int lo_j = l_s3 - (s5 + S.dlo), hi_j = f_s3 - (s5 + S.dlo);
							if (hi_j < lo_j)
								continue;
							vsel = V & (hi_j >= 63 ? ~0ull : ((1ull << (hi_j + 1)) - 1)) & (~0ull << lo_j);
							if (vsel != 0)
								break;
						}
						if (vsel == 0) {
							GM_RETURN();
							break;
						}
						L_FR(L, s, 0) = pk16(sd, lsd);
						if (S.next_s >= 0)
							L_ZD(L, S.next_s) = pk16(sd + 1, dl);
						if (e.scope == 0) {
							const int *sc = &PV.scopes[e.scopes];
							for (int k = 1; k < e.n_scopes; k++) {
								const int d1 = sc[k];
								if (PV.elems[d1].type == GM_H5) {
									unmark(L, d1);
									L_ZD(L, PV.elems[d1].searchno) = pk16(z, sd);
								}
							}
						}
						L_FR(L, s, 4) = pk16(s5, s5);
						L_FR(L, s, 2) = pk16(s5, 0);
						L_FR(L, s, 5) = pk16(l_s3, i_minl);
						L_FR(L, s, 6) = pk16(l_s3 - 1, s5 + S.dlo);
						L_FR(L, s, 7) = (uint32_t)vsel;
						L_FR(L, s, 8) = (uint32_t)(vsel >> 32);
						ph = PH_PK_S3;
					} else if (ph == PH_PK_SD) {
						const uint32_t zd = L_ZD(L, s);
						const int z = lo16(zd), dl = hi16(zd);
						const uint32_t w0 = L_FR(L, s, 0);
						const int sd = lo16(w0) - 1, lsd = hi16(w0);
						if (sd < lsd) {
							GM_RETURN();
							break;
						}
						L_FR(L, s, 0) = pk16(sd, lsd);
						if (S.next_s >= 0)
							L_ZD(L, S.next_s) = pk16(sd + 1, dl);
						if (e.scope == 0) {
							const int *sc = &PV.scopes[e.scopes];
							for (int k = 1; k < e.n_scopes; k++) {
								const int d1 = sc[k];
								if (PV.elems[d1].type == GM_H5) {
									unmark(L, d1);
									L_ZD(L, PV.elems[d1].searchno) = pk16(z, sd);
								}
							}
						}
						const int slen = sd - z + 1;
						const uint32_t w9 = L_FR(L, s, 9), w10 = L_FR(L, s, 10);
						const int p_minl = lo16(w9), p_maxl = hi16(w9);
						const int r_minl = lo16(w10), r_maxl = hi16(w10);
						if (p_maxl + r_maxl < slen)
							continue;
						int f_s5 = z + p_minl;
						int l_s5 = z + min(p_maxl, slen - r_minl);
						if (e.scope == 1) {
							const uint32_t w13 = L_FR(L, s, 13);
							const int iL_last = lo16(L_FR(L, s, 15));
							f_s5 = max(f_s5, iL_last - hi16(w13) - S.maxlen + 1);
							l_s5 = min(l_s5, iL_last - lo16(w13) - S.minlen + 1);
						}
						L_FR(L, s, 4) = pk16(f_s5 - 1, l_s5);
						ph = PH_PK_S5;
					} else if (ph == PH_PK_S5) {
						const uint32_t w4 = L_FR(L, s, 4);
// ... 259 lines not shown
```

rnamotif_b200/csrc/gm_search.cuh:

```cuda
#pragma once

#include <stddef.h>
#include <stdint.h>
#include "gpumotif_plan.h"

template <typename T>
__device__ __forceinline__ T *gm_sh(T *p)
{
	__builtin_assume(__isShared((const void *)p));
	return p;
}

namespace gm {

enum { K_SS = 0, K_WC = 1, K_PK = 2, K_PH = 3, K_TR = 4, K_QU = 5 };

struct DevSearch {
	int kind;
	int d;
	int d3;
	int loop;
	int next_s;
	int minlen, maxlen;
	int minglen, maxglen;
	int minilen, maxilen;
	int ends, pfrac, mplim;
	unsigned duplex;
	int lentab;
	int rx5, rx3;
	int mm5;
	int hmm;
	int dupi_t;
	int last;
	int fr;
	int dupi;
	int flt;
	int kid_t, kid_off;
	int sib_t, sib_off;
	int lk_t, lk_off;
	int dlo, dhi;
	int nest;
	int n_probe;
	unsigned probe[4];
	int pkm_off, pkm_n;
};
static_assert(sizeof(DevSearch) == 41 * 4, "DevSearch is staged with an odd word stride");

#define GM_MAX_DUPS 8
#define GM_MAX_CHAIN 40
#define GM_MAX_PKM 64

struct DevParams {
	int n_searches, n_descr;
	int n_pairsets, n_regex, n_scopes, n_lentab, n_sites;
	int w_winsize;
	int dminlen;
	int strict_helices;
	int halo;
	int tile;
	int words_per_lane;
	int frame_words;
	int win_stride;
	int win_stage;
	int win_bits;
	int n_dups;
	unsigned dups[GM_MAX_DUPS];
	int refill_min;
	int dfs_refill;
	int pf_search;
	int pf_z;
	int sieve;
	int pf_deep;
	int sv_helix;
	int sv_two;
	int sv_id;
	int pk_m[GM_MAX_PKM];
	int chain;
	unsigned chain_w0[GM_MAX_CHAIN];
	unsigned chain_w1[GM_MAX_CHAIN];
	int lit_present;
	int lit_rx, lit_lmin, lit_lmax, lit_mm, lit_len;
	int lite;
	int elsrc[GM_MAX_DESCR];
};

#define GM_FW_SS 2
#define GM_FW_HX 7
#define GM_FW_QU 9
#define GM_FW_PK 18

__device__ __forceinline__ uint32_t pk16(int a, int b)
{
	return (uint32_t)(a & 0xffff) | ((uint32_t)b << 16);
}
__device__ __forceinline__ int lo16(uint32_t w) { return (int)(short)(w & 0xffff); }
__device__ __forceinline__ int hi16(uint32_t w) { return (int)w >> 16; }

__device__ __forceinline__ int bcode_of(int v) { return v >> 4; }
__device__ __forceinline__ int icode_of(int v) { return v & 15; }

__device__ __forceinline__ int paired(unsigned duplex, int v5, int v3)
{
	return (duplex >> (bcode_of(v5) * 5 + bcode_of(v3))) & 1u;
}

struct DevRegex {
	int32_t n_items, bol, eol, npos, closure_iters, mm_len;
	uint64_t skip, star, dot;
	uint64_t B[16];
};
static_assert(sizeof(DevRegex) == offsetof(gm_regex_t, items), "DevRegex mirrors the head of gm_regex_t");

struct PlanView {
	DevParams par;
	const gm_elem_t *elems;
	const gm_pairset_t *pairsets;
	const DevRegex *regex;
	const int32_t *scopes;
	const uint8_t *lentab;
	const gm_site_t *sites;
	gm_ctxel_t lctx, rctx;
	int n_sites, n_pairsets, n_regex, pad_;
};

struct Lane {
	const PlanView *P;
	uint32_t *st;
	int nt;
	const uint8_t *sq;
	const DevSearch *ds;
	const gm_pairset_t *ps;
	int NS, ND;
	int el_base;
	int szero;
	int slen;
	int comp;
	uint32_t rec;
	uint32_t seq;
};

#define L_ZD(L, s)     gm_sh((L).st)[(s) * (L).nt]
#define L_FR(L, s, k)  gm_sh((L).st)[((L).NS + gm_sh((L).ds)[s].fr + (k)) * (L).nt]
#define L_EL(L, d)     gm_sh((L).st)[((L).el_base + (d)) * (L).nt]
#define L_EM(L, d)     gm_sh((L).st)[((L).el_base + (L).ND + (d)) * (L).nt]

__device__ __forceinline__ void mark(Lane &L, int d, int off, int len)
{
	L_EL(L, d) = pk16(off, len);
}
__device__ __forceinline__ void unmark(Lane &L, int d)
{
	L_EL(L, d) = pk16(GM_UNDEF, GM_UNDEF);
}
__device__ uint32_t el_word_lite(const Lane &L, int d);
__device__ __forceinline__ uint32_t el_word(const Lane &L, int d, bool lite)
{
	return lite ? el_word_lite(L, d) : L_EL(L, d);
}
__device__ __forceinline__ void set_cnt(Lane &L, int d, int mpr, int mm)
{
	L_EM(L, d) = pk16(mpr, mm);
}
__device__ __forceinline__ void set_mpr(Lane &L, int d, int mpr)
{
	L_EM(L, d) = pk16(mpr, hi16(L_EM(L, d)));
}

__device__ __noinline__ int rx_match(const DevRegex &rx_, const uint8_t *s_, int n)
{
	const DevRegex &rx = rx_;
	const uint8_t *s = s_;
	const uint64_t skip = rx.skip, star = rx.star;
	const uint64_t accept = (uint64_t)1 << rx.npos;
	const int iters = rx.closure_iters;
	uint64_t a0 = 1;
	for (int i = 0; i < iters; i++)
		a0 |= (a0 & skip) << 1;
	uint64_t a = a0;
	bool any = (a & accept) != 0;
	const bool bol = rx.bol != 0, eol = rx.eol != 0;
	if (!eol && any)
		return 1;
	for (int j = 0; j < n; j++) {
		uint64_t m = a & rx.B[icode_of(s[j])];
		a = (m << 1) | (m & star);
		for (int i = 0; i < iters; i++)
			a |= (a & skip) << 1;
		if (!bol)
			a |= a0;
		if (a & accept) {
			if (!eol)
				return 1;
		}
		if (a == 0)
			return 0;
	}
	return (a & accept) != 0 ? 1 : 0;
}

__device__ __noinline__ int rx_match_mm(const DevRegex &rx_, const uint8_t *s_, int n, int l_mm, int *n_mm)
{
	const DevRegex &rx = rx_;
	const uint8_t *s = s_;
	const int m = rx.mm_len;
	const int last = rx.bol ? 0 : n;
	int cnt = 0;
	for (int p1 = 0; p1 <= last; p1++) {
		cnt = 0;
		bool ok = true;
		for (int k = 0; k < m; k++) {
			if (p1 + k >= n) { ok = false; break; }
			uint64_t bit = (uint64_t)1 << k;
			if (!(rx.dot & bit) && !(rx.B[icode_of(s[p1 + k])] & bit)) {
				if (++cnt > l_mm) { ok = false; break; }
			}
		}
		if (ok && rx.eol && p1 + m != n)
			ok = false;
		if (ok) {
			*n_mm = cnt;
			return 1;
		}
	}
	*n_mm = cnt;
	return 0;
}

__device__ __forceinline__ int triple(const gm_pairset_t &p, int v1, int v2, int v3)
{
	int k = (bcode_of(v1) * 5 + bcode_of(v2)) * 5 + bcode_of(v3);
	return (p.multi[k >> 5] >> (k & 31)) & 1u;
}
__device__ __forceinline__ int quad(const gm_pairset_t &p, int v1, int v2, int v3, int v4)
{
	int k = ((bcode_of(v1) * 5 + bcode_of(v2)) * 5 + bcode_of(v3)) * 5 + bcode_of(v4);
	return (p.multi[k >> 5] >> (k & 31)) & 1u;
}

}
```

rnamotif_b200/csrc/gm_tilebits.h:

```cpp
#pragma once
#include <stdint.h>

#if defined(__CUDACC__)
#define GM_HD __host__ __device__ __forceinline__
#else
#define GM_HD static inline
#endif

namespace gm {

GM_HD uint32_t spread4(uint32_t h16)
{
	uint32_t t = (h16 | (h16 << 8)) & 0x00ff00ffu;
	return (t | (t << 4)) & 0x0f0f0f0fu;
}

GM_HD uint32_t gather4(uint32_t y)
{
	return ((y * 0x249u) >> 9) & 0xfu;
}

GM_HD void expand4(uint32_t t, uint32_t hb, uint32_t &fwd, uint32_t &rc)
{
	const uint32_t m7 = hb * 7u, mff = hb * 255u;
	const uint32_t lg = (((t >> 1) & 0x07070707u) - ((t >> 3) & 0x01010101u)) & m7;
	const uint32_t b = lg | ((hb ^ 0x01010101u) << 2);
	fwd = t | (b << 4);
	const uint32_t rv = ((t & 0x01010101u) << 3) | ((t & 0x02020202u) << 1) | ((t >> 1) & 0x02020202u) | ((t >> 3) & 0x01010101u);
	const uint32_t nb = 0x03030303u - lg;
	const uint32_t c = ((rv | (nb << 4)) & mff) | (0x4f4f4f4fu & ~mff);
	rc = (c >> 24) | ((c >> 8) & 0xff00u) | ((c << 8) & 0xff0000u) | (c << 24);
}

GM_HD void expand8(uint32_t x, uint32_t &f0, uint32_t &f1, uint32_t &r0, uint32_t &r1, uint32_t &bits)
{
	const uint32_t M = 0x11111111u;
	const uint32_t b0 = x & M, b1 = (x >> 1) & M, b2 = (x >> 2) & M, b3 = (x >> 3) & M;
	const uint32_t s = b0 + b1 + b2 + b3;
	const uint32_t h = s & ~(s >> 1) & M;
	const uint32_t a = b0 & h, c = b1 & h, g = b2 & h, t = b3 & h;
	bits = gather4(a & 0xffffu) | (gather4(a >> 16) << 4) | (gather4(c & 0xffffu) << 8) | (gather4(c >> 16) << 12) |
		(gather4(g & 0xffffu) << 16) | (gather4(g >> 16) << 20) | (gather4(t & 0xffffu) << 24) | (gather4(t >> 16) << 28);
	uint32_t rlo, rhi;
	expand4(spread4(x & 0xffffu), spread4(h & 0xffffu), f0, rlo);
	expand4(spread4(x >> 16), spread4(h >> 16), f1, rhi);
	r0 = rhi;
	r1 = rlo;
}

}
```

rnamotif_b200/csrc/gpumotif.cu:

```cuda
#include <cuda_runtime.h>
#include <algorithm>
#include <chrono>
#include <cstdarg>
#include <cstdio>
#include <cstdlib>
#include <cmath>
#include <cstring>
#include <condition_variable>
#include <mutex>
#include <numeric>
#include <thread>
#include <vector>

#include <cub/device/device_radix_sort.cuh>
#include <nvtx3/nvToolsExt.h>

#include "gpumotif.h"
#include "gm_machine.cuh"
#include "gm_fastn.cuh"
#include "gm_fastq.cuh"
#include "gm_hostpack.h"

using namespace gm;

static thread_local char g_err[512] = "";
struct gm_ctx;

static int fail(const char *fmt, ...)
{
	va_list ap;
	va_start(ap, fmt);
	vsnprintf(g_err, sizeof g_err, fmt, ap);
	va_end(ap);
	return -1;
}

#define CU(call)                                                                        \
	do {                                                                                \
		cudaError_t e_ = (call);                                                        \
		if (e_ != cudaSuccess)                                                          \
			return fail("%s: %s (%s:%d)", #call, cudaGetErrorString(e_), __FILE__, __LINE__); \
	} while (0)

struct NvtxRange {
	explicit NvtxRange(const char *name) { nvtxRangePushA(name); }
	~NvtxRange() { nvtxRangePop(); }
};

#define GM_PACK_SLOTS 4

enum DbKind { DB_NONE, DB_CHARS, DB_HOSTPACK, DB_2BIT, DB_FASTN, DB_FASTQ };

struct gm_ctx {
	gm_plan_t plan;
	DevParams par;
	DevSearch ds[GM_MAX_DESCR];
	int device;
	int n_sm;
	cudaStream_t stream;
	cudaStream_t copy_stream;
	cudaStream_t pack_stream;
	std::vector<cudaEvent_t> cp_ev;
	cudaEvent_t ev[6];
	std::vector<cudaEvent_t> chunk_ev;
	std::vector<int64_t> chunk_end;
	bool upload_fresh;
	cudaEvent_t up_ev[2];
	PackTeam *team;
	std::thread up_thread;
	std::mutex up_m;
	std::condition_variable up_cv;
	int up_published;
	char up_err[256];
	uint8_t *h_slot[GM_PACK_SLOTS];
	size_t slot_cap;
	cudaEvent_t slot_ev[GM_PACK_SLOTS];
	gm_plan_t *d_plan;
	DevSearch *d_ds;
	gm_score_t *d_score;
	DbKind db;
	uint8_t *d_chars;
	size_t chars_cap;
	uint8_t *d_packed;
	size_t packed_cap;
	int64_t *d_rec_off;
	size_t rec_cap;
	std::vector<int64_t> rec_off;
	int64_t total_nt;
	std::vector<uint64_t> start_pre;
	uint8_t *d_text;
	size_t text_cap;
	int64_t *d_hdr_off;
	size_t hdr_cap;
	void *d_fsum, *d_fstart;
	size_t fsum_cap, fstart_cap;
	std::vector<int64_t> hdr_off;
	const uint8_t *d_seq_chars;
	int64_t *d_tb;
	size_t tb_cap;
	std::vector<int64_t> tb;
	uint8_t *d_gz;
	size_t gz_cap;
	void *d_bgzf;
	size_t bgzf_cap;
	std::vector<BgzfMember> bgzf;
	uint8_t *d_win, *h_win;
	size_t win_cap, h_win_cap;
	std::vector<uint8_t> wins;
	unsigned long long *d_counters;
	uint32_t *d_hits;
	size_t hit_cap;
	int stride_words;
	int threads, blocks;
	size_t smem_bytes;
	bool use_split;
	bool full;
	int a_threads, a_blocks, b_threads, b_blocks;
	size_t a_smem, b_smem;
	uint32_t *d_wl;
	size_t wl_cap;
	int64_t seg_nt;
	std::vector<uint32_t> hits;
	uint32_t *h_raw;
	size_t h_raw_cap;
	std::vector<uint64_t> keys;
	void *d_sort;
	size_t sort_cap;
	uint32_t *d_sorted;
	size_t sorted_cap;
	bool dev_sorted;
	std::vector<cudaEvent_t> seg_ev;
	int n_seg_ev;
	const uint32_t *hits_view;
	size_t n_hits;
	size_t n_raw;
	gm_scan_stats_t stats;
	bool pending;
	int64_t p_begin, p_end;
	int p_strands;
};

extern "C" const char *gm_last_error(void) { return g_err; }
extern "C" const char *gm_version(void) { return "libgpumotif 0.1 (sm_100a)"; }

extern "C" int gm_host_alloc(void **out, size_t n_bytes)
{
	if (out == NULL)
		return fail("out is NULL");
	*out = NULL;
	CU(cudaMallocHost(out, n_bytes ? n_bytes : 1));
	return 0;
}
extern "C" void gm_host_free(void *p)
{
	if (p != NULL)
		cudaFreeHost(p);
}

extern "C" int gm_device_count(void)
{
	int n = 0;
	if (cudaGetDeviceCount(&n) != cudaSuccess) {
		cudaGetLastError();
		return 0;
	}
	return n;
}

typedef void (*search_kernel_t)(const ScanArgs);
static search_kernel_t fused_kernel(bool full, int pf)
{
	if (pf == 2)
		return full ? (search_kernel_t)gm_search_kernel<0, true, 2> : (search_kernel_t)gm_search_kernel<0, false, 2>;
	if (pf == 1)
		return full ? (search_kernel_t)gm_search_kernel<0, true, 1> : (search_kernel_t)gm_search_kernel<0, false, 1>;
	return full ? (search_kernel_t)gm_search_kernel<0, true, 0> : (search_kernel_t)gm_search_kernel<0, false, 0>;
}
static int pf_of(const DevParams &par)
{
	return par.sieve ? 2 : par.lit_present ? 1 : 0;
}
static int pre_pf(const DevParams &par)
{
	return par.sieve && par.sv_two ? 3 : pf_of(par);
}
static search_kernel_t dfs_kernel(bool full)
{
	return full ? (search_kernel_t)gm_dfs_kernel<true> : (search_kernel_t)gm_dfs_kernel<false>;
}
static search_kernel_t pre_kernel(int pf)
{
	return pf == 3 ? (search_kernel_t)gm_filter_kernel<3> : pf == 2 ? (search_kernel_t)gm_filter_kernel<2> :
		pf == 1 ? (search_kernel_t)gm_filter_kernel<1> : (search_kernel_t)gm_filter_kernel<0>;
}

#define GM_SMEM_OPTIN (227 * 1024)


#define GM_WL_SEG_NT ((int64_t)16 << 20)

static size_t wl_entries()
{
	const char *e = getenv("GPUMOTIF_WL_CAP");
	if (e != NULL && atoll(e) >= 1024)
		return (size_t)atoll(e);
	return (size_t)GM_WL_SEG_NT * 2;
}
static int64_t wl_safe_seg()
{
	return (int64_t)(wl_entries() / 2);
}

static int kind_of(const gm_plan_t *pl, int d)
{
	const gm_elem_t &e = pl->elems[d];
	switch (e.type) {
	case GM_SS: return K_SS;
	case GM_H5: return e.proper ? K_WC : K_PK;
	case GM_P5: return K_PH;
	case GM_T1: return K_TR;
	case GM_Q1: return K_QU;
	}
	return -1;
}

static int check_plan(const gm_plan_t *pl, DevSearch *ds, DevParams *par)
{
	if (pl == NULL)
		return fail("plan is NULL");
	if (pl->magic != GM_PLAN_MAGIC || pl->version != GM_PLAN_VERSION)
		return fail("not a gm_plan_t of version %d", GM_PLAN_VERSION);
	const int NS = pl->n_searches, ND = pl->n_descr;
	if (ND <= 0 || ND > GM_MAX_DESCR || NS <= 0 || NS > ND)
		return fail("plan: %d elements / %d searches out of range", ND, NS);
	if (pl->n_regex < 0 || pl->n_regex > GM_MAX_REGEX || pl->n_pairsets < 0 ||
	    pl->n_pairsets > GM_MAX_PAIRSET || pl->n_sites < 0 || pl->n_sites > GM_MAX_SITES ||
	    pl->n_scopes < 0 || pl->n_scopes > GM_MAX_SCOPES || pl->n_lentab < 0 || pl->n_lentab > GM_LENTAB_SIZE)
		return fail("plan: table sizes out of range");
	if (pl->dminlen <= 0)
		return fail("plan: descriptor can match the empty string (dminlen = %d)", pl->dminlen);
	if (pl->dmaxlen == GM_UNBOUNDED && pl->windowsize > 16000)
		return fail("plan: unbounded descriptor with windowsize %d > 16000", pl->windowsize);
	const int W = pl->dmaxlen < pl->windowsize ? pl->dmaxlen : pl->windowsize;
	if (W > 16000)
		return fail("plan: window of %d nt exceeds the device limit of 16000", W);
	int cx = 0;
	if (pl->lctx.present)
		cx = std::max(cx, pl->lctx.maxlen);
	if (pl->rctx.present)
		cx = std::max(cx, pl->rctx.maxlen);
	if (cx > 4000)
		return fail("plan: context of %d nt exceeds the device limit of 4000", cx);

	for (int d = 0; d < ND; d++) {
		const gm_elem_t &e = pl->elems[d];
		if (e.type < 0 || e.type >= GM_N_TYPES)
			return fail("element %d: bad type %d", d, e.type);
		if (e.maxlen == GM_UNBOUNDED || e.maxlen < 0 || e.minlen < 0 || e.maxlen > 32000)
			return fail("element %d: length range [%d,%d] not supported", d, e.minlen, e.maxlen);
		if (e.regex >= pl->n_regex || e.pairset >= pl->n_pairsets)
			return fail("element %d: table index out of range", d);
		if (e.type != GM_SS && e.regex >= 0 && e.minlen == 0)
			return fail("element %d: seq= on a helix with minlen=0 is undefined in the reference "
				    "(src/find_motif.c:986-1021 reads an unset candidate)", d);
		if (e.type != GM_SS && e.maxlen > GM_MAX_HLEN)
			return fail("element %d: helix maxlen %d > %d", d, e.maxlen, GM_MAX_HLEN);
		if (e.regex >= 0 && pl->regex[e.regex].npos > GM_RE_MAX_POS)
			return fail("element %d: regex too long", d);
	}

	memset(ds, 0, sizeof(DevSearch) * GM_MAX_DESCR);
	for (int s = 0; s < NS; s++) {
		const int d = pl->searches[s];
		if (d < 0 || d >= ND)
			return fail("search %d: bad element %d", s, d);
		const gm_elem_t &e = pl->elems[d];
		DevSearch &S = ds[s];
		if (e.searchno != s)
			return fail("search %d: element %d says searchno %d", s, d, e.searchno);
		S.kind = kind_of(pl, d);
		if (S.kind < 0)
			return fail("search %d: element %d of type %d cannot head a search", s, d, e.type);
		S.d = d;
		S.d3 = -1;
		S.loop = e.next >= 0 ? 1 : (e.outer < 0 ? 1 : 0);
		S.next_s = -1;
		if (e.next >= 0) {
			S.next_s = pl->elems[e.next].searchno;
			if (S.next_s <= s || S.next_s >= NS)
				return fail("search %d: successor search %d out of order", s, S.next_s);
		}
		S.minlen = e.minlen; S.maxlen = e.maxlen;
		S.minglen = e.minglen; S.maxglen = e.maxglen;
		S.minilen = e.minilen; S.maxilen = e.maxilen;
		if (S.loop && (e.maxglen == GM_UNBOUNDED || e.maxglen < 0 || e.minglen < 0))
			return fail("search %d: unbounded group length", s);
		S.ends = e.ends; S.pfrac = e.pfrac; S.mplim = e.mplim;
		S.duplex = e.pairset >= 0 ? pl->pairsets[e.pairset].duplex : 0;
		S.lentab = e.lentab;
		S.rx5 = e.regex;
		S.rx3 = -1;
		S.mm5 = e.mismatch;
		S.last = s == NS - 1;
		if (S.kind != K_SS) {
			const int need = S.kind == K_TR ? 2 : S.kind == K_QU ? 3 : 1;
			if (e.n_mates != need)
				return fail("search %d: element %d has %d mates, expected %d", s, d, e.n_mates, need);
			for (int k = 0; k < need; k++)
				if (e.mates[k] <= d || e.mates[k] >= ND)
					return fail("search %d: bad mate", s);
			S.d3 = e.mates[need - 1];
			S.rx3 = pl->elems[S.d3].regex;
			S.hmm = (e.regex >= 0 && e.mismatch > 0) ||
				(S.rx3 >= 0 && pl->elems[S.d3].mismatch > 0);
			if (e.pairset < 0)
				return fail("search %d: helix without a pairset", s);
			if (S.pfrac && e.lentab < 0)
				return fail("search %d: pairfrac without a length table", s);
			if ((S.kind == K_TR && e.mptab < 0) ||
			    (S.kind == K_QU && pl->elems[e.mates[0]].mptab < 0))
				return fail("search %d: missing mispair-by-length table", s);
			if (S.kind == K_TR && pl->pairsets[e.pairset].n_bases != 3)
				return fail("search %d: triplex needs a 3-base pairset", s);
			if (S.kind == K_QU && pl->pairsets[pl->elems[e.mates[0]].pairset].n_bases != 4)
				return fail("search %d: quadruplex needs a 4-base pairset", s);
		}
		if (S.last && S.kind != K_SS)
			return fail("the last search must be a single-strand element");
		if (S.kind == K_WC || S.kind == K_PH || S.kind == K_TR || S.kind == K_QU) {
			if (e.inner < 0 || pl->elems[e.inner].searchno != s + 1)
				return fail("search %d: helix without an interior (the reference dereferences "
					    "NULL there, src/find_motif.c:453-454) or interior not searched next", s);
		}
		if (S.kind == K_TR) {
			const gm_elem_t &e1 = pl->elems[e.mates[0]];
			if (e1.inner < 0 || pl->elems[e1.inner].searchno <= s + 1)
				return fail("search %d: triplex second interior missing", s);
		}
		if (S.kind == K_QU) {
			for (int k = 0; k < 2; k++) {
				const gm_elem_t &ek = pl->elems[e.mates[k]];
				if (ek.inner < 0 || pl->elems[ek.inner].searchno <= s + 1)
					return fail("search %d: quadruplex interior %d missing", s, k + 2);
			}
// ... 351 lines not shown
					if (ok) {
						st.cm = cm;
						st.both = p5 && p3;
						st.con = 1;
						st.bud = bud;
						any_con = true;
					}
				}
			}
			if (!st.con && !steps.empty() && !steps.back().con) {
				steps.back().mn += st.mn;
				steps.back().mx = (int)std::min<long>((long)steps.back().mx + st.mx, 4095);
			} else
				steps.push_back(st);
			if (steps.back().mx > 4095)
				steps.back().mx = 4095;
		}
		bool fits = any_con && (int)steps.size() <= GM_MAX_CHAIN;
		long span = 0;
		for (const Step &st : steps) {
			if (st.mn > 4095)
				fits = false;
			span += st.mx - st.mn;
		}
		if (span > 4096)
			fits = false;
		if (fits) {
			par->chain = (int)steps.size();
			for (size_t i = 0; i < steps.size(); i++) {
				const Step &st = steps[i];
				par->chain_w0[i] = (unsigned)st.mn | ((unsigned)st.mx << 12) | ((unsigned)st.cm << 24) |
					((unsigned)st.both << 28) | ((unsigned)st.con << 29);
				par->chain_w1[i] = st.bud;
			}
			if (!par->sieve)
				par->sieve = 1;
			double est = 1.0;
			for (const Step &st : steps) {
				const double choices = (double)(st.mx - st.mn + 1);
				if (!st.con) {
					est = std::min(1.0, est * choices);
					continue;
				}
				int nb = 0;
				for (int x = 0; x < 4; x++)
					nb += (st.cm >> x) & 1;
				const double q = nb / 4.0;
				const int b0 = (int)(st.bud & 3u), L0 = st.mn;
				double pr = 0, c = 1;
				for (int k = 0; k <= std::min(b0, L0); k++) {
					pr += c * pow(q, L0 - k) * pow(1 - q, k);
					c = c * (L0 - k) / (k + 1);
				}
				est = std::min(1.0, std::min(1.0, pr) * std::min(1.0, est * choices));
			}
			chain_est = std::min(1.0, est);
		}
	}
	if (par->sieve && par->sv_helix && par->pf_search >= 0 && !par->pf_deep && !par->sv_two &&
	    getenv("GPUMOTIF_NO_TWO_STAGE") == NULL) {
		double est = 1.0;
		if (par->lit_present) {
			const int L0 = par->lit_len, mm = par->lit_mm;
			double pr = 0, c = 1;
			for (int k = 0; k <= std::min(mm, L0); k++) {
				pr += c * pow(0.25, L0 - k) * pow(0.75, k);
				c = c * (L0 - k) / (k + 1);
			}
			est = std::min(1.0, pr * (par->lit_lmax - par->lit_lmin + 1));
		}
		if (par->chain)
			est *= chain_est;
		const double bar = par->chain && !par->lit_present ? 0.2 : 0.08;
		if (est < bar || getenv("GPUMOTIF_TWO_STAGE") != NULL)
			par->sv_two = 1;
		if (getenv("GPUMOTIF_DEBUG") != NULL)
			fprintf(stderr, "gpumotif: stage-1 share estimate %.4f (literal %d, chain %d steps, chain share %.4f)\n", est,
				par->lit_present, par->chain, chain_est);
	}
	par->lite = 1;
	for (int s = 0; s < NS; s++)
		if ((ds[s].kind != K_SS && ds[s].kind != K_WC) || ds[s].hmm)
			par->lite = 0;
	{
		const int flt0 = par->pf_search >= 0 ? ds[par->pf_search].flt : 0;
		const bool strong = par->pf_search >= 0 && ((flt0 >> 8) & 0xff) == 0 && (flt0 & 0xff) >= 3;
		par->refill_min = !par->lite ? 4 : strong ? GM_REFILL_MIN : 8;
	}
	par->dfs_refill = par->lite ? 24 : 16;
	if (getenv("GPUMOTIF_REFILL") != NULL)
		par->refill_min = par->dfs_refill = std::max(1, std::min(32, atoi(getenv("GPUMOTIF_REFILL"))));
	for (int d = 0; d < ND; d++) {
		const gm_elem_t &e = pl->elems[d];
		int src = e.searchno;
		if (e.type == GM_H3 && e.n_mates >= 1)
			src = pl->elems[e.mates[0]].searchno;
		par->elsrc[d] = src >= 0 && src < NS ? src : 0;
	}
	par->words_per_lane = NS + fr + (par->lite ? 0 : 2) * ND;
	return 0;
}

extern "C" int gm_plan_check(const gm_plan_t *plan)
{
	static thread_local DevSearch ds[GM_MAX_DESCR];
	DevParams par;
	return check_plan(plan, ds, &par);
}

extern "C" int gm_plan_describe(const gm_plan_t *plan, char *out, size_t cap)
{
	static thread_local DevSearch ds[GM_MAX_DESCR];
	DevParams par;
	if (out == NULL || cap == 0)
		return fail("bad argument");
	out[0] = 0;
	if (check_plan(plan, ds, &par))
		return -1;
	size_t n = 0;
	auto put = [&](const char *fmt, ...) {
		if (n + 1 >= cap)
			return;
		va_list ap;
		va_start(ap, fmt);
		int k = vsnprintf(out + n, cap - n, fmt, ap);
		va_end(ap);
		if (k > 0)
			n = std::min(cap - 1, n + (size_t)k);
	};
	static const char *kn[] = {"ss", "wc", "pk", "ph", "tr", "qu"};
	put("window %d halo %d lite %d n_dups %d refill %d\n", par.w_winsize, par.halo, par.lite, par.n_dups, par.refill_min);
	put("level0: pf_search %d pf_z %d sieve %d two-stage %d helix-term %d deep %d literal %d (len %d at %d..%d mm %d) chain %d\n", par.pf_search,
	    par.pf_z, par.sieve, par.sv_two, par.sv_helix, par.pf_deep, par.lit_present, par.lit_len, par.lit_lmin, par.lit_lmax, par.lit_mm,
	    par.chain);
	for (int s = 0; s < par.n_searches; s++) {
		const DevSearch &S = ds[s];
		put("search %2d %s d %d d3 %d loop %d next %d len %d..%d D %d..%d req %d budget %d first %d dup %d/%d", s, kn[S.kind], S.d, S.d3,
		    S.loop, S.next_s, S.minlen, S.maxlen, S.dlo, S.dhi, S.flt & 0xff, (S.flt >> 8) & 0xff, (S.flt >> 16) & 1, S.dupi, S.dupi_t);
		if (S.kid_t >= 0)
			put(" kid %d+%d%s", S.kid_t, S.kid_off, (S.nest & 1) ? "" : " (not nested)");
		if (S.sib_t >= 0)
			put(" sib %d+%d", S.sib_t, S.sib_off);
		if (S.lk_t >= 0)
			put(" tail %d-%d", S.lk_t, S.lk_off);
		for (int i = 0; i < S.n_probe; i++)
			put(" probe(%s off %u len %u rx %u mm %u)", (S.probe[i] & 3) == 0 ? "after-5'" : (S.probe[i] & 3) == 1 ? "after-3'" : "before-3'",
			    (S.probe[i] >> 2) & 1023, (S.probe[i] >> 12) & 255, (S.probe[i] >> 20) & 31, (S.probe[i] >> 25) & 15);
		put("\n");
	}
	return 0;
}


static size_t smem_need(const gm_ctx *c, int threads, int tile, bool with_state = true)
{
	const int Lb = (tile + 2 * c->par.halo + 31) & ~31;
	const size_t stage = ((Lb >> 1) + 32 + 15) & ~15;
	const size_t pb = (((size_t)2 * c->par.n_dups * 4 * (((Lb + 31) >> 5) + 4) * 4) + 15) & ~(size_t)15;
	const size_t lit = c->par.lit_present ? (((size_t)2 * (((Lb + 31) >> 5) + 4) * 4) + 15) & ~(size_t)15 : 0;
	const size_t buf_bytes = 2 * (size_t)Lb + pb + (GM_REC_CACHE + 2) * 8 + lit;
	const size_t warp_bytes = 16 + stage + (with_state ? 2 : 1) * buf_bytes + GM_QCAP * 2 +
		(c->par.sieve ? ((6 * (size_t)(((Lb + 31) >> 5) + 4) * 4 + 15) & ~(size_t)15) : 0) +
		(c->par.chain ? ((6 * (size_t)(((Lb + 31) >> 5) + 4) * 4 + 15) & ~(size_t)15) : 0);
	size_t n = plan_smem_bytes(c->par);
	n += c->par.lit_present ? 16 * 8 : 0;
	n += (size_t)(threads >> 5) * warp_bytes;
	if (with_state)
		n += (size_t)c->par.words_per_lane * threads * 4;
	return n;
}

static size_t dfs_smem_need(const gm_ctx *c, int threads)
{
	size_t n = plan_smem_bytes(c->par);
	n += (size_t)threads * c->par.win_stride;
	n += (size_t)threads * c->par.win_bits * 4;
	n += (size_t)c->par.words_per_lane * threads * 4;
	return n;
}

static int warps_per_sm(gm_ctx *c, int threads, int tile)
{
	const size_t need = smem_need(c, threads, tile);
	if (need + 1024 > 227 * 1024)
		return 0;
	int n = 0;
	if (cudaFuncSetAttribute(fused_kernel(c->full, pf_of(c->par)), cudaFuncAttributeMaxDynamicSharedMemorySize, GM_SMEM_OPTIN) != cudaSuccess ||
	    cudaOccupancyMaxActiveBlocksPerMultiprocessor(&n, fused_kernel(c->full, pf_of(c->par)), threads, need) != cudaSuccess) {
		cudaGetLastError();
		return 0;
	}
	return n * threads / 32;
}

static int auto_tile(gm_ctx *c)
{
	int best_tile = 256;
	double best = -1;
	for (int tile = 256; tile <= 2048; tile += 64) {
		int w = 0;
		for (int t = 64; t <= 256; t <<= 1)
			w = std::max(w, warps_per_sm(c, t, tile));
		const double score = w * (double)tile / (tile + 2.0 * c->par.halo);
		if (score > best * 1.001) {
			best = score;
			best_tile = tile;
		}
	}
	return best_tile;
}

static int configure_launch(gm_ctx *c, int tile)
{
	const int tile_arg = tile;
	if (tile <= 0)
		tile = auto_tile(c);
	const size_t smem_sm = 227 * 1024;
	int best_t = 0;
	size_t best_warps = 0;
	for (int t = 64; t <= 256; t <<= 1) {
		size_t warps = (size_t)warps_per_sm(c, t, tile);
		if (warps > best_warps) {
			best_warps = warps;
			best_t = t;
		}
	}
	if (best_t == 0 && smem_need(c, 32, tile) + 1024 <= smem_sm)
		best_t = 32;
	if (best_t == 0)
		return fail("plan needs %zu bytes of shared memory per 32-lane block (limit %zu)",
			    smem_need(c, 32, tile), smem_sm);
	c->threads = best_t;
	c->par.tile = tile;
	c->smem_bytes = smem_need(c, best_t, tile);
	CU(cudaFuncSetAttribute(fused_kernel(c->full, pf_of(c->par)), cudaFuncAttributeMaxDynamicSharedMemorySize, GM_SMEM_OPTIN));
	int per_sm = 0;
	CU(cudaOccupancyMaxActiveBlocksPerMultiprocessor(&per_sm, fused_kernel(c->full, pf_of(c->par)), c->threads, c->smem_bytes));
	if (per_sm < 1)
		return fail("search kernel does not fit on an SM (threads %d, smem %zu)", c->threads, c->smem_bytes);
	c->blocks = per_sm * c->n_sm;
	if (getenv("GPUMOTIF_DEBUG") != NULL)
		fprintf(stderr, "gpumotif: tile %d, %d threads x %d blocks (%d per SM), %zu bytes smem per block, %s kernel\n",
			tile, c->threads, c->blocks, per_sm, c->smem_bytes, c->full ? "full" : "lite");

	const DevSearch &S0 = c->ds[0];
	const int wtot = c->par.halo * 2 - c->par.w_winsize;
	int words = (wtot + 3) / 4;
	if (!(words & 1))
		words++;
	c->par.win_stride = words * 4;
	c->par.win_stage = (((wtot + 1) / 2 + 1 + 15 + 15) & ~15);
	c->par.win_bits = (c->par.n_dups * 4 * (((wtot + 31) >> 5) + 3)) | 1;
	bool eligible = wtot <= 512 &&
		(c->par.pf_search >= 0 || c->par.lit_present ||
		 (S0.rx5 >= 0 && S0.mm5 == 0 && !c->plan.regex[S0.rx5].eol));
	const char *force = getenv("GPUMOTIF_PATH");
	if (force != NULL && strcmp(force, "split") == 0)
		eligible = wtot <= 512;
	else if (force != NULL && strcmp(force, "fused") == 0)
		eligible = false;
	else
	{
		double est = 1.0;
		if (c->par.sieve && c->par.sv_helix && c->par.pf_search >= 0) {
			const DevSearch &T = c->ds[c->par.pf_search];
			int allowed = 0;
			for (int x = 0; x < 4; x++)
				for (int y = 0; y < 4; y++)
					allowed += (T.duplex >> (x * 5 + y)) & 1u;
			const double q = allowed / 16.0;
			const int req = T.flt & 0xff, budget = (T.flt >> 8) & 0xff;
			double pr = pow(q, req);
			if (budget >= 1)
				pr += req * (1 - q) * pow(q, req - 1);
			est = std::min(1.0, (T.dhi - T.dlo + 1) * pr);
		}
		const bool strong = c->par.pf_deep || c->par.chain || c->par.lit_present || est <= 0.5;
		eligible = wtot <= 512 && ((c->par.sieve && strong) || (c->par.lit_present && c->full));
	}
	const int fused_tile0 = c->par.tile;
	if (eligible && tile_arg <= 0 && c->par.sieve) {
		for (int t2 = 1984; t2 >= 448; t2 = t2 == 1984 ? 960 : 448) {
			if (smem_need(c, 256, t2, false) * 2 + 2048 <= smem_sm) {
				tile = t2;
				break;
			}
			if (t2 == 448)
				break;
		}
		c->par.tile = tile;
	}
	const int fused_tile = fused_tile0;
	c->use_split = false;
	if (eligible) {
		c->a_threads = 256;
		c->a_smem = smem_need(c, c->a_threads, tile, false);
		int best_w = 0;
		c->b_threads = 0;
		for (int t = 64; t <= 256; t <<= 1) {
			size_t need = dfs_smem_need(c, t);
			if (need > smem_sm)
				continue;
			int n = 0;
			if (cudaFuncSetAttribute(dfs_kernel(c->full), cudaFuncAttributeMaxDynamicSharedMemorySize, GM_SMEM_OPTIN) != cudaSuccess ||
			    cudaOccupancyMaxActiveBlocksPerMultiprocessor(&n, dfs_kernel(c->full), t, need) != cudaSuccess)
				continue;
			if (n * t > best_w) {
				best_w = n * t;
				c->b_threads = t;
				c->b_smem = need;
				c->b_blocks = n * c->n_sm;
			}
		}
		cudaGetLastError();
		int na = 0;
		if (c->b_threads > 0 && c->a_smem <= smem_sm &&
		    cudaFuncSetAttribute(pre_kernel(pre_pf(c->par)), cudaFuncAttributeMaxDynamicSharedMemorySize, GM_SMEM_OPTIN) == cudaSuccess &&
		    cudaFuncSetAttribute(dfs_kernel(c->full), cudaFuncAttributeMaxDynamicSharedMemorySize, GM_SMEM_OPTIN) == cudaSuccess &&
		    cudaOccupancyMaxActiveBlocksPerMultiprocessor(&na, pre_kernel(pre_pf(c->par)), c->a_threads, c->a_smem) == cudaSuccess &&
		    na >= 1) {
			c->a_blocks = na * c->n_sm;
			c->use_split = true;
		}
		cudaGetLastError();
	}
	if (!c->use_split)
		c->par.tile = fused_tile;
	if (getenv("GPUMOTIF_DEBUG") != NULL && c->use_split)
		fprintf(stderr, "gpumotif: split path, tile %d, sieve/prefilter %d x %d (%zu B), dfs %d x %d (%zu B)\n", c->par.tile,
			c->a_blocks, c->a_threads, c->a_smem, c->b_blocks, c->b_threads, c->b_smem);
	return 0;
}

extern "C" int gm_ctx_create(gm_ctx **out, const gm_plan_t *plan, int device)
{
	if (out == NULL)
		return fail("out is NULL");
	*out = NULL;
	gm_ctx *c = new gm_ctx();
	memset(&c->stats, 0, sizeof c->stats);
	c->d_chars = c->d_packed = NULL;
	c->d_plan = NULL;
	c->d_ds = NULL;
	c->d_score = NULL;
	c->d_text = NULL;
	c->d_hdr_off = NULL;
	c->d_fsum = c->d_fstart = NULL;
	c->text_cap = c->hdr_cap = c->fsum_cap = c->fstart_cap = 0;
	c->d_seq_chars = NULL;
	c->d_tb = NULL;
	c->tb_cap = 0;
	c->db = DB_NONE;
	c->d_gz = NULL;
	c->d_bgzf = NULL;
	c->gz_cap = c->bgzf_cap = 0;
	c->d_win = c->h_win = NULL;
	c->win_cap = c->h_win_cap = 0;
	c->d_rec_off = NULL;
	c->d_counters = NULL;
	c->d_hits = NULL;
	c->d_wl = NULL;
	c->wl_cap = 0;
	c->h_raw = NULL;
	c->h_raw_cap = 0;
	c->d_sort = NULL;
	c->sort_cap = 0;
	c->d_sorted = NULL;
	c->sorted_cap = 0;
	c->dev_sorted = false;
	c->hits_view = NULL;
	c->n_seg_ev = 0;
	c->seg_nt = getenv("GPUMOTIF_SEG_NT") != NULL && atoll(getenv("GPUMOTIF_SEG_NT")) > 0 ? atoll(getenv("GPUMOTIF_SEG_NT")) : wl_safe_seg();
	c->use_split = false;
	c->chars_cap = c->packed_cap = c->rec_cap = 0;
	c->total_nt = 0;
	c->n_hits = 0;
	c->pending = false;
	c->stream = NULL;
	if (check_plan(plan, c->ds, &c->par)) {
		delete c;
		return -1;
	}
	c->plan = *plan;
	c->full = !c->par.lite;
	int n = gm_device_count();
	if (n <= 0) {
		delete c;
		return fail("no CUDA device: libgpumotif has no CPU path");
	}
	if (device < 0 || device >= n) {
		delete c;
		return fail("device %d out of range (%d visible)", device, n);
	}
	c->device = device;
	for (int i = 0; i < 6; i++)
		c->ev[i] = NULL;
	cudaDeviceProp prop;
	cudaError_t e = cudaSetDevice(device);
	if (e == cudaSuccess)
		e = cudaGetDeviceProperties(&prop, device);
	if (e != cudaSuccess) {
		delete c;
		return fail("cudaSetDevice(%d): %s", device, cudaGetErrorString(e));
	}
	if (prop.major != 10) {
		delete c;
		return fail("device %d is sm_%d%d; this library is built for sm_100a only", device, prop.major, prop.minor);
	}
	c->n_sm = prop.multiProcessorCount;
	c->stride_words = (int)((sizeof(gm_hit_hdr_t) + plan->n_descr * sizeof(gm_hit_el_t)) / 4);
	c->hit_cap = (size_t)1 << 20;
	c->copy_stream = NULL;
	c->pack_stream = NULL;
	c->upload_fresh = false;
	c->up_ev[0] = c->up_ev[1] = NULL;
	c->team = NULL;
	c->up_published = -1;
	c->up_err[0] = 0;
	c->slot_cap = 0;
	for (int i = 0; i < GM_PACK_SLOTS; i++) {
		c->h_slot[i] = NULL;
		c->slot_ev[i] = NULL;
	}
	if (cudaStreamCreateWithFlags(&c->stream, cudaStreamNonBlocking) != cudaSuccess ||
	    cudaStreamCreateWithFlags(&c->copy_stream, cudaStreamNonBlocking) != cudaSuccess) {
		delete c;
		return fail("cudaStreamCreate failed");
	}
	{
		int lo_pri = 0, hi_pri = 0;
		cudaDeviceGetStreamPriorityRange(&lo_pri, &hi_pri);
		if (cudaStreamCreateWithPriority(&c->pack_stream, cudaStreamNonBlocking, hi_pri) != cudaSuccess) {
			gm_ctx_destroy(c);
			return fail("cudaStreamCreateWithPriority failed");
		}
	}
	cudaEventCreate(&c->up_ev[0]);
	cudaEventCreate(&c->up_ev[1]);
	for (int i = 0; i < 6; i++)
		cudaEventCreate(&c->ev[i]);
	if (cudaMalloc(&c->d_counters, 32 * sizeof(unsigned long long)) != cudaSuccess) {
		gm_ctx_destroy(c);
		return fail("cudaMalloc(counters) failed");
	}
	if (cudaMalloc(&c->d_plan, sizeof(gm_plan_t)) != cudaSuccess ||
	    cudaMalloc(&c->d_ds, sizeof(DevSearch) * GM_MAX_DESCR) != cudaSuccess ||
	    cudaMemcpyAsync(c->d_plan, &c->plan, sizeof c->plan, cudaMemcpyHostToDevice, c->stream) != cudaSuccess ||
	    cudaMemcpyAsync(c->d_ds, c->ds, sizeof(DevSearch) * GM_MAX_DESCR, cudaMemcpyHostToDevice, c->stream) != cudaSuccess) {
		gm_ctx_destroy(c);
		return fail("plan upload failed: %s", cudaGetErrorString(cudaGetLastError()));
	}
	if (configure_launch(c, 0)) {
		gm_ctx_destroy(c);
		return -1;
	}
	if (cudaStreamSynchronize(c->stream) != cudaSuccess) {
		gm_ctx_destroy(c);
		return fail("plan upload failed: %s", cudaGetErrorString(cudaGetLastError()));
	}
	*out = c;
	return 0;
}

extern "C" void gm_ctx_destroy(gm_ctx *c)
{
	if (c == NULL)
		return;
	cudaSetDevice(c->device);
	if (c->up_thread.joinable())
		c->up_thread.join();
	delete c->team;
	if (c->stream)
		cudaStreamSynchronize(c->stream);
	if (c->copy_stream)
		cudaStreamSynchronize(c->copy_stream);
	if (c->pack_stream)
		cudaStreamSynchronize(c->pack_stream);
	for (cudaEvent_t e : c->cp_ev)
		cudaEventDestroy(e);
	for (int i = 0; i < GM_PACK_SLOTS; i++) {
		if (c->slot_ev[i])
			cudaEventDestroy(c->slot_ev[i]);
		cudaFreeHost(c->h_slot[i]);
// ... 911 lines not shown
		return fail("the device holds no characters after gm_db_upload_chars_hostpack (the caller has them)");
	return c->db == DB_2BIT ? 1 : 0;
}

extern "C" int gm_db_get_chars(gm_ctx *c, int64_t off, int64_t n, char *out)
{
	if (c == NULL || out == NULL || off < 0 || n < 0)
		return fail("bad argument");
	const int codes = char_source(c);
	if (codes < 0)
		return -1;
	if (off + n > c->total_nt)
		return fail("range [%lld, %lld) outside the %lld uploaded nucleotides", (long long)off, (long long)(off + n),
			    (long long)c->total_nt);
	CU(cudaSetDevice(c->device));
	if (sync_uploads(c))
		return -1;
	if (codes) {
		if (n == 0)
			return 0;
		const int64_t b0 = off >> 1, b1 = (off + n + 1) >> 1;
		std::vector<uint8_t> pk((size_t)(b1 - b0));
		CU(cudaMemcpy(pk.data(), c->d_packed + b0, pk.size(), cudaMemcpyDeviceToHost));
		for (int64_t i = 0; i < n; i++) {
			const int64_t g = off + i;
			out[i] = "?acmgrsvtwyhkdbn"[(pk[(size_t)((g >> 1) - b0)] >> (4 * (g & 1))) & 15];
		}
		return 0;
	}
	if (n > 0)
		CU(cudaMemcpy(out, c->d_seq_chars + off, (size_t)n, cudaMemcpyDeviceToHost));
	for (int64_t i = 0; i < n; i++) {
		unsigned ch = (unsigned char)out[i] | 0x20;
		out[i] = ch == 'u' ? 't' : (char)ch;
	}
	return 0;
}

extern "C" int64_t gm_db_total_nt(const gm_ctx *c) { return c == NULL ? -1 : c->db == DB_NONE ? 0 : c->total_nt; }


static int launch(gm_ctx *c)
{
	NvtxRange nvtx_("gpumotif: launch sieve / enumeration kernels");
	if (c->d_hits == NULL) {
		CU(cudaMalloc(&c->d_hits, c->hit_cap * (size_t)c->stride_words * 4));
	}
	CU(cudaMemsetAsync(c->d_counters, 0, 32 * sizeof(unsigned long long), c->stream));
	ScanArgs A;
	A.par = c->par;
	A.plan = c->d_plan;
	A.ds = c->d_ds;
	A.packed = c->d_packed;
	A.total_nt = c->total_nt;
	A.rec_off = c->d_rec_off;
	A.n_rec = (int)c->rec_off.size() - 1;
	A.g_begin = c->p_begin;
	A.g_end = c->p_end;
	A.strands = c->p_strands;
	A.n_tiles = (c->p_end - c->p_begin + c->par.tile - 1) / c->par.tile;
	A.tile_counter = c->d_counters + 0;
	A.hit_count = c->d_counters + 1;
	A.start_count = c->d_counters + 2;
	A.hits = c->d_hits;
	A.hit_cap = c->hit_cap;
	A.stride_words = c->stride_words;
	A.wl = NULL;
	A.wl_count = c->d_counters + 3;
	A.wl_head = c->d_counters + 4;
	A.wl_cap = 0;
	CU(cudaEventRecord(c->ev[3], c->stream));
	c->n_seg_ev = 0;
	const int n_chunks = (int)c->chunk_end.size();
	if (A.n_tiles > 0 && !c->use_split && c->upload_fresh && n_chunks > 1 && n_chunks <= 16) {
		int64_t lo = c->p_begin;
		for (int i = 0; i < n_chunks && lo < c->p_end; i++) {
			int64_t hi = i == n_chunks - 1 ? c->p_end : std::min<int64_t>(c->p_end, c->chunk_end[i] - c->par.halo - c->par.tile);
			if (wait_published(c, i))
				return -1;
			CU(cudaStreamWaitEvent(c->stream, c->chunk_ev[i], 0));
			if (hi <= lo)
				continue;
			if (i != n_chunks - 1)
				hi = lo + (hi - lo) / c->par.tile * c->par.tile;
			if (hi <= lo)
				continue;
			A.g_begin = lo;
			A.g_end = hi;
			A.n_tiles = (hi - lo + c->par.tile - 1) / c->par.tile;
			A.tile_counter = c->d_counters + 8 + i;
			int blocks = (int)std::min<int64_t>(c->blocks, A.n_tiles);
			fused_kernel(c->full, pf_of(c->par))<<<blocks, c->threads, c->smem_bytes, c->stream>>>(A);
			CU(cudaGetLastError());
			c->stats.n_launches++;
			lo = hi;
		}
	} else if (A.n_tiles > 0 && !c->use_split) {
		if (n_chunks > 0) {
			if (wait_published(c, n_chunks - 1))
				return -1;
			CU(cudaStreamWaitEvent(c->stream, c->chunk_ev[n_chunks - 1], 0));
		}
		int blocks = (int)std::min<int64_t>(c->blocks, A.n_tiles);
		fused_kernel(c->full, pf_of(c->par))<<<blocks, c->threads, c->smem_bytes, c->stream>>>(A);
		CU(cudaGetLastError());
		c->stats.n_launches++;
	} else if (A.n_tiles > 0) {
		const bool stream_in = c->upload_fresh && n_chunks > 1 && n_chunks <= 16;
		if (n_chunks > 0 && !stream_in) {
			if (wait_published(c, n_chunks - 1))
				return -1;
			CU(cudaStreamWaitEvent(c->stream, c->chunk_ev[n_chunks - 1], 0));
		}
		const size_t need = wl_entries();
		const int64_t seg = std::min<int64_t>(c->seg_nt, c->p_end - c->p_begin);
		if (c->d_wl == NULL || c->wl_cap < need) {
			cudaFree(c->d_wl);
			c->d_wl = NULL;
			CU(cudaMalloc(&c->d_wl, need * GM_WL_WORDS * 4));
			c->wl_cap = need;
		}
		A.wl = c->d_wl;
		A.wl_cap = c->wl_cap;
		int ci = 0;
		int64_t seg_end = c->p_begin;
		for (int64_t g0 = c->p_begin; g0 < c->p_end; g0 = A.g_end) {
			if (g0 == seg_end) {
				seg_end = std::min<int64_t>(g0 + seg, c->p_end);
				CU(cudaMemsetAsync(c->d_counters + 3, 0, 2 * sizeof(unsigned long long), c->stream));
			}
			A.g_begin = g0;
			A.g_end = seg_end;
			if (stream_in) {
				const int64_t slack = (int64_t)c->par.halo + c->par.tile;
				while (ci < n_chunks - 1 && c->chunk_end[ci] - slack <= g0)
					ci++;
				if (wait_published(c, ci))
					return -1;
				CU(cudaStreamWaitEvent(c->stream, c->chunk_ev[ci], 0));
				if (ci < n_chunks - 1)
					A.g_end = std::min<int64_t>(A.g_end, c->chunk_end[ci] - slack);
				if (seg_end - A.g_end <= 2 * slack)
					seg_end = A.g_end;
			}
			A.n_tiles = (A.g_end - A.g_begin + c->par.tile - 1) / c->par.tile;
			CU(cudaMemsetAsync(c->d_counters + 0, 0, sizeof(unsigned long long), c->stream));
			int ablocks = (int)std::min<int64_t>(c->a_blocks, A.n_tiles);
			while ((int)c->seg_ev.size() < 2 * (c->n_seg_ev + 1)) {
				cudaEvent_t e;
				CU(cudaEventCreate(&e));
				c->seg_ev.push_back(e);
			}
			CU(cudaEventRecord(c->seg_ev[2 * c->n_seg_ev], c->stream));
			pre_kernel(pre_pf(c->par))<<<ablocks, c->a_threads, c->a_smem, c->stream>>>(A);
			CU(cudaGetLastError());
			CU(cudaEventRecord(c->seg_ev[2 * c->n_seg_ev + 1], c->stream));
			c->n_seg_ev++;
			c->stats.n_launches++;
			if (A.g_end == seg_end) {
				dfs_kernel(c->full)<<<c->b_blocks, c->b_threads, c->b_smem, c->stream>>>(A);
				CU(cudaGetLastError());
				c->stats.n_launches++;
			}
		}
	}
	CU(cudaEventRecord(c->ev[4], c->stream));
	c->upload_fresh = false;
	return 0;
}

extern "C" int gm_scan_launch(gm_ctx *c, int64_t g_begin, int64_t g_end, int strands)
{
	if (c == NULL)
		return fail("ctx is NULL");
	if (c->pending)
		return fail("a scan is already in flight");
	if (strands != 1 && strands != 2)
		return fail("strands must be 1 or 2");
	if (c->db == DB_NONE)
		return fail("no database uploaded");
	if (g_begin < 0 || g_end > c->total_nt || g_begin > g_end)
		return fail("range [%lld, %lld) outside the database of %lld nt", (long long)g_begin,
			    (long long)g_end, (long long)c->total_nt);
	CU(cudaSetDevice(c->device));
	c->p_begin = g_begin;
	c->p_end = g_end;
	c->p_strands = strands;
	c->stats.n_launches = 0;
	c->stats.n_retries = 0;
	c->stats.kernel_ms = 0;
	c->stats.filter_ms = 0;
	c->stats.n_survivors = 0;
	c->stats.n_filter_launches = 0;
	if (launch(c))
		return -1;
	c->pending = true;
	return 0;
}

struct HitKey {
	uint32_t rec, comp, szero, seq;
	uint32_t idx;
};

__global__ void gm_sortkey_kernel(const uint32_t *__restrict__ hits, unsigned long long n, int sw,
	unsigned long long *__restrict__ keys, uint32_t *__restrict__ idx)
{
	for (unsigned long long i = blockIdx.x * (unsigned long long)blockDim.x + threadIdx.x; i < n;
	     i += (unsigned long long)gridDim.x * blockDim.x) {
		const uint32_t *h = hits + i * sw;
		keys[i] = (h[3] >> 31) ? ~0ull : ((unsigned long long)h[0] << 32) | ((unsigned long long)(h[3] & 1) << 31) |
			(unsigned long long)(h[1] & 0x7fffffffu);
		idx[i] = (uint32_t)i;
	}
}
__global__ void gm_gather_kernel(const uint32_t *__restrict__ hits, const uint32_t *__restrict__ idx,
	unsigned long long n, int sw, uint32_t *__restrict__ out)
{
	const unsigned long long total = n * sw;
	for (unsigned long long k = blockIdx.x * (unsigned long long)blockDim.x + threadIdx.x; k < total;
	     k += (unsigned long long)gridDim.x * blockDim.x) {
		const unsigned long long i = k / sw;
		out[k] = hits[(unsigned long long)idx[i] * sw + (k - i * sw)];
	}
}

extern "C" int gm_scan_finish(gm_ctx *c)
{
	if (c == NULL)
		return fail("ctx is NULL");
	if (!c->pending)
		return fail("no scan in flight");
	c->pending = false;
	CU(cudaSetDevice(c->device));
	unsigned long long cnt[8];
	nvtxRangePushA("gpumotif: wait for the kernels");
	struct PopOnce { bool done = false; void pop() { if (!done) { nvtxRangePop(); done = true; } } ~PopOnce() { pop(); } } wait_range;
	for (;;) {
		CU(cudaMemcpyAsync(cnt, c->d_counters, sizeof cnt, cudaMemcpyDeviceToHost, c->stream));
		CU(cudaStreamSynchronize(c->stream));
		float ms = 0;
		cudaEventElapsedTime(&ms, c->ev[3], c->ev[4]);
		c->stats.kernel_ms += ms;
		for (int i = 0; i < c->n_seg_ev; i++) {
			float f = 0;
			if (cudaEventElapsedTime(&f, c->seg_ev[2 * i], c->seg_ev[2 * i + 1]) == cudaSuccess)
				c->stats.filter_ms += f;
		}
		c->stats.n_filter_launches += (uint32_t)c->n_seg_ev;
		c->stats.n_survivors += cnt[6];
		if (cudaEventQuery(c->up_ev[1]) == cudaSuccess && cudaEventElapsedTime(&ms, c->up_ev[0], c->up_ev[1]) == cudaSuccess) {
			c->stats.h2d_ms = ms;
			c->stats.pack_ms = 0;
		}
		cudaGetLastError();
		if (getenv("GPUMOTIF_DEBUG") != NULL)
			fprintf(stderr, "gpumotif: hits %llu, starts %llu, worklist (last segment) %llu, machine entries %llu\n",
				cnt[1], cnt[2], cnt[3], cnt[5]);
		if (c->use_split && cnt[7]) {
			if (c->seg_nt <= wl_safe_seg())
				return fail("worklist overflow with default segments (internal error)");
			c->seg_nt = wl_safe_seg();
			c->stats.n_retries++;
			if (launch(c))
				return -1;
			continue;
		}
		if (c->use_split && c->p_end > c->p_begin) {
			const double rate = (double)cnt[6] / ((double)(c->p_end - c->p_begin) * c->p_strands);
			const double cap = (double)wl_entries();
			double seg = rate > 0 ? 0.25 * cap / (rate * c->p_strands) : 1e18;
			seg = std::max<double>((double)wl_safe_seg(), std::min<double>(seg, (double)((int64_t)1 << 30)));
			c->seg_nt = (int64_t)seg / wl_safe_seg() * wl_safe_seg();
		}
		if (cnt[1] <= c->hit_cap)
			break;
		if ((double)cnt[1] * c->stride_words * 4 > 48e9)
			return fail("%llu candidates in this range need %.1f GB of hit buffer: scan a smaller range "
				    "(gm_scan(ctx, lo, hi, ...)) or tighten the descriptor",
				    cnt[1], (double)cnt[1] * c->stride_words * 4 / 1e9);
		c->stats.n_retries++;
		cudaFree(c->d_hits);
		c->d_hits = NULL;
		c->hit_cap = (size_t)cnt[1] + (size_t)cnt[1] / 16 + 1024;
		if (launch(c))
			return -1;
	}
	wait_range.pop();
	NvtxRange nvtx_("gpumotif: order + gather candidates");
	const size_t n_all = (size_t)cnt[1];
	const size_t sw = (size_t)c->stride_words;
	size_t n_rej = 0;
	if (c->d_score != NULL && n_all > 0) {
		NvtxRange nvtx_s("gpumotif: score pre-screen");
		CU(cudaMemsetAsync(c->d_counters + 30, 0, sizeof(unsigned long long), c->stream));
		const int sblocks = (int)std::min<size_t>((n_all + 127) / 128, (size_t)c->n_sm * 32);
		gm_score_kernel<<<sblocks, 128, 0, c->stream>>>(c->d_hits, n_all, (int)sw, c->d_score, c->d_plan, c->d_packed,
			c->d_rec_off, c->d_counters + 30);
		CU(cudaGetLastError());
		unsigned long long rej = 0;
		CU(cudaMemcpyAsync(&rej, c->d_counters + 30, sizeof rej, cudaMemcpyDeviceToHost, c->stream));
		CU(cudaStreamSynchronize(c->stream));
		n_rej = (size_t)rej;
	}
	const size_t n = n_all - n_rej;
	if (n_all * sw > c->h_raw_cap) {
		cudaFreeHost(c->h_raw);
// ... 196 lines not shown
```

Measured before the change: 113.3.

## Add packed-nibble sieve filter kernel that drops expanded sequence copies from shared memory

Adds a packed variant of the split-path filter kernel. It no longer expands the tile into forward and reverse-complement byte copies in shared memory. Instead it reads sequence characters on demand through a nibble view over the TMA staging buffer, which it rewrites in place. Regex, probe and mask helpers are templated on the sequence view. Host setup picks the tile size and thread count for this kernel by an occupancy-times-efficiency score. The goal is to cut per-warp shared memory so more warps fit on each SM, at the cost of extra decode work on every character access and an added async proxy fence.

```diff
diff --git a/profiles/summarize_abf.py b/profiles/summarize_abf.py
--- /dev/null
+++ b/profiles/summarize_abf.py
@@ -0,0 +1,30 @@
+import json
+import sys
+
+out, rounds, libs = sys.argv[1], int(sys.argv[2]), sys.argv[3:]
+rows = {}
+for lib in libs:
+    for r in range(1, rounds + 1):
+        try:
+            j = json.loads(open(f"{out}/abf_{lib}_{r}.json").read().strip().splitlines()[-1])
+        except Exception as e:
+            print(f"{lib} round {r}: no result ({e})")
+            continue
+        rows.setdefault(("trna (headline)", lib), []).append((j["value"], j["e2e"]["value"], j["roofline"]["kernel_ms"]))
+        for e in j.get("per_config", []):
+            rows.setdefault((e["config"], lib), []).append((e["value"], e["e2e"]["value"], e["filter_ms_per_step"]))
+
+
+def med(xs):
+    xs = sorted(x for x in xs if x is not None)
+    return (xs[len(xs) // 2], xs[-1] - xs[0]) if xs else (float("nan"), float("nan"))
+
+
+print(f"{'workload':24s} {'lib':6s} {'resident':>16s} {'e2e':>16s} {'filter ms/step':>18s}  (median +- spread over rounds)")
+for wl in dict.fromkeys(k[0] for k in rows):
+    for lib in libs:
+        v = rows.get((wl, lib))
+        if not v:
+            continue
+        (a, da), (b, db), (c, dc) = (med([x[i] for x in v]) for i in range(3))
+        print(f"{wl:24s} {lib:6s} {a:9.2f} +-{da:5.2f} {b:9.2f} +-{db:5.2f} {c:11.3f} +-{dc:5.3f}")
diff --git a/rnamotif_b200/csrc/gm_kernel.cuh b/rnamotif_b200/csrc/gm_kernel.cuh
--- a/rnamotif_b200/csrc/gm_kernel.cuh
+++ b/rnamotif_b200/csrc/gm_kernel.cuh
@@ -218,6 +218,10 @@
 {
 	asm volatile("mbarrier.arrive.expect_tx.shared::cta.b64 _, [%0], %1;" ::"r"(smem_u32(bar)), "r"(bytes)
 		: "memory");
+}
+__device__ __forceinline__ void fence_proxy_async()
+{
+	asm volatile("fence.proxy.async.shared::cta;" ::: "memory");
 }
 __device__ __forceinline__ void tma_bulk_g2s(void *dst, const void *src, uint32_t bytes, uint64_t *bar)
 {
diff --git a/rnamotif_b200/csrc/gm_machine.cuh b/rnamotif_b200/csrc/gm_machine.cuh
--- a/rnamotif_b200/csrc/gm_machine.cuh
+++ b/rnamotif_b200/csrc/gm_machine.cuh
@@ -1,5 +1,6 @@
 #pragma once
 
+#include <type_traits>
 #include "gm_kernel.cuh"
 #include "gm_tilebits.h"
 
@@ -87,7 +88,8 @@
 	int n_dups;
 };
 
-__device__ __forceinline__ uint64_t wc_mask_body(const PairBits &pb, const uint8_t *sq, int strand, int sqbase,
+template <typename Seq>
+__device__ __forceinline__ uint64_t wc_mask_body(const PairBits &pb, Seq sq, int strand, int sqbase,
 	int dupi, int flt, int z, int lo, int n)
 {
 	const uint64_t ones = n >= 64 ? ~0ull : ((1ull << n) - 1);
@@ -123,7 +125,8 @@
 	return (budget == 0 ? a0 : budget == 1 ? a1 : a2) & ones;
 }
 
-__device__ __noinline__ uint64_t wc_mask(const PairBits &pb, const uint8_t *sq, int strand, int sqbase,
+template <typename Seq>
+__device__ __noinline__ uint64_t wc_mask(const PairBits &pb, Seq sq, int strand, int sqbase,
 	int dupi, int flt, int z, int lo, int n)
 {
 	return wc_mask_body(pb, sq, strand, sqbase, dupi, flt, z, lo, n);
@@ -212,7 +215,8 @@
 	return __funnelshift_r(set[q >> 5], set[(q >> 5) + 1], q & 31);
 }
 
-__device__ __noinline__ uint64_t wc_mask_rev(const PairBits &pb, const uint8_t *sq, int strand, int sqbase,
+template <typename Seq>
+__device__ __noinline__ uint64_t wc_mask_rev(const PairBits &pb, Seq sq, int strand, int sqbase,
 	int dupi_t, int flt, int e, int zlo, int n)
 {
 	const uint64_t ones = n >= 64 ? ~0ull : ((1ull << n) - 1);
@@ -238,7 +242,8 @@
 	return (budget == 0 ? a0 : budget == 1 ? a1 : a2) & ones;
 }
 
-__device__ __forceinline__ bool tail_feasible(const PairBits &pb, const uint8_t *sq, int strand, int sqbase,
+template <typename Seq>
+__device__ __forceinline__ bool tail_feasible(const PairBits &pb, Seq sq, int strand, int sqbase,
 	const DevSearch &S, const DevSearch &T, int s5, int s3, int hl)
 {
 	const int e = s3 - hl - S.lk_off;
@@ -263,7 +268,8 @@
 		}                                                                \
 	} while (0)
 
-__device__ __noinline__ bool probes_ok(const Lane &L, const DevSearch &S, int s5, int s3, int hl, int wend)
+template <typename Seq>
+__device__ __noinline__ bool probes_ok(const Lane &L, Seq sq, const DevSearch &S, int s5, int s3, int hl, int wend)
 {
 	for (int i = 0; i < S.n_probe; i++) {
 		const unsigned pr = S.probe[i];
@@ -274,13 +280,13 @@
 			return false;
 		const DevRegex &rx = PV.regex[rxi];
 		int n_mm;
-		if (mm > 0 ? !rx_match_mm(rx, L.sq + pos, len, mm, &n_mm) : !rx_match(rx, L.sq + pos, len))
+		if (mm > 0 ? !rx_match_mm(rx, sq + pos, len, mm, &n_mm) : !rx_match(rx, sq + pos, len))
 			return false;
 	}
 	return true;
 }
 
-template <int MODE, bool FULL, int PF>
+template <int MODE, bool FULL, int PF, bool PACKED = false>
 __device__ __forceinline__ void gm_search_body(const ScanArgs &A)
 {
 	constexpr bool SIEVE = PF >= 2;
@@ -295,11 +301,12 @@
 	const int nwb = ((Lbytes + 31) >> 5) + 4;
 	const int n_dups = A.par.n_dups;
 	const int NBUF = MODE == 0 ? 2 : 1;
+	const int seq_bytes = PACKED ? 0 : 2 * Lbytes;
 
 	const int nwarps = nt >> 5;
 	const size_t pb_bytes = (((size_t)2 * n_dups * 4 * nwb * 4) + 15) & ~(size_t)15;
 	const size_t lit_bytes = LIT ? (((size_t)2 * nwb * 4) + 15) & ~(size_t)15 : 0;
-	const size_t buf_bytes = 2 * (size_t)Lbytes + pb_bytes + (GM_REC_CACHE + 2) * 8 + lit_bytes;
+	const size_t buf_bytes = (size_t)seq_bytes + pb_bytes + (GM_REC_CACHE + 2) * 8 + lit_bytes;
 	const bool CHAIN = SIEVE && A.par.chain > 0;
 	const size_t warp_bytes = 16 + (size_t)stage_bytes + NBUF * buf_bytes + GM_QCAP * 2 + (SIEVE ? ((6 * (size_t)nwb * 4 + 15) & ~(size_t)15) : 0) +
 		(CHAIN ? ((6 * (size_t)nwb * 4 + 15) & ~(size_t)15) : 0);
@@ -381,9 +388,9 @@
 		uint8_t *bp = bufs + (size_t)b * buf_bytes;
 		sm_fwd = bp;
 		sm_rc = bp + Lbytes;
-		pb.base = reinterpret_cast<uint32_t *>(bp + 2 * (size_t)Lbytes);
-		sm_rec = reinterpret_cast<int64_t *>(bp + 2 * (size_t)Lbytes + pb_bytes);
-		sm_lit = reinterpret_cast<uint32_t *>(bp + 2 * (size_t)Lbytes + pb_bytes + (GM_REC_CACHE + 2) * 8);
+		pb.base = reinterpret_cast<uint32_t *>(bp + seq_bytes);
+		sm_rec = reinterpret_cast<int64_t *>(bp + seq_bytes + pb_bytes);
+		sm_lit = reinterpret_cast<uint32_t *>(bp + seq_bytes + pb_bytes + (GM_REC_CACHE + 2) * 8);
 		gA = A.g_begin + t * (int64_t)TILE;
 		gB = min(gA + (int64_t)TILE, A.g_end);
 		lo = gA - H;
@@ -392,6 +399,8 @@
 		const int64_t bs = (lo_c >> 1) & ~(int64_t)15;
 		const uint32_t nbytes = (uint32_t)((((hi_c + 1) >> 1) - bs + 15) & ~(int64_t)15);
 		if (lane == 0) {
+			if (PACKED)
+				fence_proxy_async();
 			mbar_expect_tx(&sm->bar, nbytes);
 			tma_bulk_g2s(sm_stage, A.packed + bs, nbytes, &sm->bar);
 			int a = 0, bb = A.n_rec;
@@ -417,34 +426,57 @@
 		uint32_t *pbw = const_cast<uint32_t *>(pb.base);
 		const int nw = Lbytes >> 5;
 		{
-			const uint32_t *stw = reinterpret_cast<const uint32_t *>(sm_stage);
-			const int n_stw = stage_bytes >> 2;
-			const int base_q = (int)(lo - 2 * bs);
-			const int sh = (base_q & 7) * 4;
-			const bool edge = lo < 0 || lo + Lbytes > A.total_nt;
-			const unsigned sel1 = (lane & 1) ? 0x3715u : 0x6240u, sel2 = (lane & 2) ? 0x3276u : 0x5410u;
-			for (int i0 = lane * 8; i0 < ((Lbytes + 255) & ~255); i0 += 256) {
-				const int wq = (base_q + i0) >> 3;
-				const uint32_t w0 = stw[min(max(wq, 0), n_stw - 1)], w1 = stw[min(max(wq + 1, 0), n_stw - 1)];
-				uint32_t x = __funnelshift_r(w0, w1, sh);
-				if (edge) {
-					const int64_t g0 = lo + i0;
-					const int klo = (int)min((int64_t)8, max((int64_t)0, -g0));
-					const int khi = (int)min((int64_t)8, max((int64_t)0, A.total_nt - g0));
-					const uint32_t m_hi = khi >= 8 ? ~0u : ((1u << (4 * khi)) - 1u);
-					const uint32_t m_lo = klo >= 8 ? 0u : (~0u << (4 * klo));
-					x &= m_hi & m_lo;
-				}
-				uint32_t f0, f1, r0, r1, bits;
-				expand8(x, f0, f1, r0, r1, bits);
-				uint32_t o = __shfl_xor_sync(0xffffffffu, bits, 1);
-				bits = __byte_perm(bits, o, sel1);
-				o = __shfl_xor_sync(0xffffffffu, bits, 2);
-				bits = __byte_perm(bits, o, sel2);
-				if (i0 < Lbytes) {
-					*reinterpret_cast<uint2 *>(sm_fwd + i0) = make_uint2(f0, f1);
-					*reinterpret_cast<uint2 *>(sm_rc + Lbytes - 8 - i0) = make_uint2(r0, r1);
-					pbw[(size_t)(lane & 3) * nwb + (i0 >> 5)] = bits;
+			if constexpr (!PACKED) {
+				const uint32_t *stw = reinterpret_cast<const uint32_t *>(sm_stage);
+				const int n_stw = stage_bytes >> 2;
+				const int base_q = (int)(lo - 2 * bs);
+				const int sh = (base_q & 7) * 4;
+				const bool edge = lo < 0 || lo + Lbytes > A.total_nt;
+				const unsigned sel1 = (lane & 1) ? 0x3715u : 0x6240u, sel2 = (lane & 2) ? 0x3276u : 0x5410u;
+				for (int i0 = lane * 8; i0 < ((Lbytes + 255) & ~255); i0 += 256) {
+					const int wq = (base_q + i0) >> 3;
+					const uint32_t w0 = stw[min(max(wq, 0), n_stw - 1)], w1 = stw[min(max(wq + 1, 0), n_stw - 1)];
+					uint32_t x = __funnelshift_r(w0, w1, sh);
+					if (edge) {
+						const int64_t g0 = lo + i0;
+						const int klo = (int)min((int64_t)8, max((int64_t)0, -g0));
+						const int khi = (int)min((int64_t)8, max((int64_t)0, A.total_nt - g0));
+						const uint32_t m_hi = khi >= 8 ? ~0u : ((1u << (4 * khi)) - 1u);
+						const uint32_t m_lo = klo >= 8 ? 0u : (~0u << (4 * klo));
+						x &= m_hi & m_lo;
+					}
+					uint32_t f0, f1, r0, r1, bits;
+					expand8(x, f0, f1, r0, r1, bits);
+					uint32_t o = __shfl_xor_sync(0xffffffffu, bits, 1);
+					bits = __byte_perm(bits, o, sel1);
+					o = __shfl_xor_sync(0xffffffffu, bits, 2);
+					bits = __byte_perm(bits, o, sel2);
+					if (i0 < Lbytes) {
+						*reinterpret_cast<uint2 *>(sm_fwd + i0) = make_uint2(f0, f1);
+						*reinterpret_cast<uint2 *>(sm_rc + Lbytes - 8 - i0) = make_uint2(r0, r1);
+						pbw[(size_t)(lane & 3) * nwb + (i0 >> 5)] = bits;
+					}
+				}
+			} else {
+				uint32_t *stw = reinterpret_cast<uint32_t *>(sm_stage);
+				const int n_stw = stage_bytes >> 2;
+				const int base_q = (int)(lo - 2 * bs);
+				const unsigned sel1 = (lane & 1) ? 0x3715u : 0x6240u, sel2 = (lane & 2) ? 0x3276u : 0x5410u;
+				const int n_it = (Lbytes + 255) >> 8;
+				for (int it = 0; it < n_it; it++) {
+					const int i0 = ((base_q < 0 ? n_it - 1 - it : it) << 8) + lane * 8;
+					const uint32_t x = tile_word(stw, n_stw, base_q, i0, lo, A.total_nt);
+					uint32_t f0, f1, r0, r1, bits;
+					expand8(x, f0, f1, r0, r1, bits);
+					uint32_t o = __shfl_xor_sync(0xffffffffu, bits, 1);
+					bits = __byte_perm(bits, o, sel1);
+					o = __shfl_xor_sync(0xffffffffu, bits, 2);
+					bits = __byte_perm(bits, o, sel2);
+					if (i0 < Lbytes)
+						pbw[(size_t)(lane & 3) * nwb + (i0 >> 5)] = bits;
+					__syncwarp();
+					if (i0 < Lbytes)
+						stw[i0 >> 3] = x;
 				}
 			}
 		}
@@ -505,6 +537,14 @@
 		have_tile = true;
 	};
 
+	using Seq = typename std::conditional<PACKED, NibView, const uint8_t *>::type;
+	auto seq_of = [&](int comp, int idx) -> Seq {
+		if constexpr (!PACKED)
+			return comp ? sm_rc + (Lbytes - 1 - idx) : sm_fwd + idx;
+		else
+			return NibView{sm_stage, idx, comp ? -1 : 1};
+	};
+
 	auto next_tile = [&]() -> int64_t {
 		unsigned long long t_ = 0;
 		if (lane == 0)
@@ -566,7 +606,7 @@
 			return false;
 		my_starts++;
 		const DevSearch &S0 = sm_ds[0];
-		const uint8_t *sq = comp ? sm_rc + (Lbytes - 1 - idx) : sm_fwd + idx;
+		const Seq sq = seq_of(comp, idx);
 		const int base = comp ? Lbytes - 1 - idx : idx;
 		const int dl = min(W, slen - szero) - 1;
 		if (LIT) {
@@ -611,7 +651,7 @@
 			return false;
 		const DevSearch &S0 = sm_ds[0];
 		if (S0.rx5 >= 0 && S0.mm5 == 0 && !PV.regex[S0.rx5].eol) {
-			const uint8_t *sq = comp ? sm_rc + (Lbytes - 1 - idx) : sm_fwd + idx;
+			const Seq sq = seq_of(comp, idx);
 			const int dl = min(W, slen - szero) - 1;
 			return rx_match(PV.regex[S0.rx5], sq, min(S0.maxlen, dl + 1)) != 0;
 		}
@@ -625,7 +665,7 @@
 			return false;
 		const DevSearch &S0 = sm_ds[0];
 		const DevSearch &SP = sm_ds[A.par.pf_search];
-		const uint8_t *sq = comp ? sm_rc + (Lbytes - 1 - idx) : sm_fwd + idx;
+		const Seq sq = seq_of(comp, idx);
 		const int base = comp ? Lbytes - 1 - idx : idx;
 		const int dl = min(W, slen - szero) - 1;
 		if (S0.rx5 >= 0 && S0.mm5 == 0 && !PV.regex[S0.rx5].eol &&
@@ -647,12 +687,8 @@
 						continue;
 					if (SP.lk_t >= 0 && !tail_feasible(pb, sq, comp, base, SP, sm_ds[SP.lk_t], pz, s3, hl))
 						continue;
-					if (SP.n_probe) {
-						Lane Lq = L;
-						Lq.sq = sq;
-						if (!probes_ok(Lq, SP, pz, s3, hl, dl))
-							continue;
-					}
+					if (SP.n_probe && !probes_ok(L, sq, SP, pz, s3, hl, dl))
+						continue;
 					return true;
 				}
 			}
@@ -1051,6 +1087,11 @@
 __global__ void __launch_bounds__(256, 2) gm_filter_kernel(const ScanArgs A)
 {
 	gm_search_body<1, false, PF>(A);
+}
+template <int PF>
+__global__ void __launch_bounds__(128, 5) gm_filter_packed_kernel(const ScanArgs A)
+{
+	gm_search_body<1, false, PF, true>(A);
 }
 
 template <bool FULL>
diff --git a/rnamotif_b200/csrc/gm_machine_body.inc b/rnamotif_b200/csrc/gm_machine_body.inc
--- a/rnamotif_b200/csrc/gm_machine_body.inc
+++ b/rnamotif_b200/csrc/gm_machine_body.inc
@@ -195,7 +195,7 @@
 								if (!any)
 									continue;
 							}
-							if (S.n_probe && !probes_ok(L, S, s5, s3, hl, hi16(L_ZD(L, 0))))
+							if (S.n_probe && !probes_ok(L, L.sq, S, s5, s3, hl, hi16(L_ZD(L, 0))))
 								continue;
 						}
 						L_FR(L, s, 0) = pk16(top + 1, lsd);
@@ -429,7 +429,7 @@
 								if (!any)
 									found = 0;
 							}
-							if (found > 0 && S.n_probe && !probes_ok(L, S, s5, s3, hl, hi16(L_ZD(L, 0))))
+							if (found > 0 && S.n_probe && !probes_ok(L, L.sq, S, s5, s3, hl, hi16(L_ZD(L, 0))))
 								found = 0;
 							if (found)
 								break;
diff --git a/rnamotif_b200/csrc/gm_search.cuh b/rnamotif_b200/csrc/gm_search.cuh
--- a/rnamotif_b200/csrc/gm_search.cuh
+++ b/rnamotif_b200/csrc/gm_search.cuh
@@ -166,10 +166,11 @@
 	L_EM(L, d) = pk16(mpr, hi16(L_EM(L, d)));
 }
 
-__device__ __noinline__ int rx_match(const DevRegex &rx_, const uint8_t *s_, int n)
+template <typename Seq>
+__device__ __noinline__ int rx_match(const DevRegex &rx_, Seq s_, int n)
 {
 	const DevRegex &rx = rx_;
-	const uint8_t *s = s_;
+	const Seq s = s_;
 	const uint64_t skip = rx.skip, star = rx.star;
 	const uint64_t accept = (uint64_t)1 << rx.npos;
 	const int iters = rx.closure_iters;
@@ -198,10 +199,11 @@
 	return (a & accept) != 0 ? 1 : 0;
 }
 
-__device__ __noinline__ int rx_match_mm(const DevRegex &rx_, const uint8_t *s_, int n, int l_mm, int *n_mm)
+template <typename Seq>
+__device__ __noinline__ int rx_match_mm(const DevRegex &rx_, Seq s_, int n, int l_mm, int *n_mm)
 {
 	const DevRegex &rx = rx_;
-	const uint8_t *s = s_;
+	const Seq s = s_;
 	const int m = rx.mm_len;
 	const int last = rx.bol ? 0 : n;
 	int cnt = 0;
diff --git a/rnamotif_b200/csrc/gm_tilebits.h b/rnamotif_b200/csrc/gm_tilebits.h
--- a/rnamotif_b200/csrc/gm_tilebits.h
+++ b/rnamotif_b200/csrc/gm_tilebits.h
@@ -3,8 +3,10 @@
 
 #if defined(__CUDACC__)
 #define GM_HD __host__ __device__ __forceinline__
+#define GM_HDM __host__ __device__ __forceinline__
 #else
 #define GM_HD static inline
+#define GM_HDM inline
 #endif
 
 namespace gm {
@@ -48,4 +50,43 @@
 	r1 = rlo;
 }
 
+GM_HD uint32_t tile_word(const uint32_t *stw, int n_stw, int base_q, int i0, int64_t lo, int64_t total_nt)
+{
+	const int wq = (base_q + i0) >> 3;
+	const int ia = wq < 0 ? 0 : wq > n_stw - 1 ? n_stw - 1 : wq, ib = wq + 1 < 0 ? 0 : wq + 1 > n_stw - 1 ? n_stw - 1 : wq + 1;
+	const int sh = (base_q & 7) * 4;
+#if defined(__CUDA_ARCH__)
+	uint32_t x = __funnelshift_r(stw[ia], stw[ib], sh);
+#else
+	uint32_t x = (uint32_t)((((uint64_t)stw[ib] << 32) | stw[ia]) >> sh);
+#endif
+	const int64_t g0 = lo + i0;
+	if (g0 < 0 || g0 + 8 > total_nt) {
+		const int64_t klo_ = -g0 < 0 ? 0 : -g0 > 8 ? 8 : -g0, khi_ = total_nt - g0 < 0 ? 0 : total_nt - g0 > 8 ? 8 : total_nt - g0;
+		const int klo = (int)klo_, khi = (int)khi_;
+		const uint32_t m_hi = khi >= 8 ? ~0u : ((1u << (4 * khi)) - 1u);
+		const uint32_t m_lo = klo >= 8 ? 0u : (~0u << (4 * klo));
+		x &= m_hi & m_lo;
+	}
+	return x;
 }
+
+struct NibView {
+	const uint8_t *nib;
+	int p;
+	int dir;
+
+	GM_HDM NibView operator+(int r) const { return NibView{nib, p + dir * r, dir}; }
+	GM_HDM int operator[](int r) const
+	{
+		const int q = p + dir * r;
+		const unsigned c = (nib[q >> 1] >> ((q & 1) * 4)) & 15u;
+		const bool rc = dir < 0;
+		const unsigned sh = 4 * (c & 7);
+		const uint32_t bt = (c & 8) ? (rc ? 0x44444440u : 0x44444443u) : (rc ? 0x44414234u : 0x44424104u);
+		const unsigned ic = rc ? ((((c & 8) ? 0xfffffff1u : 0xfff2f48fu) >> sh) & 15u) : c;
+		return (int)(ic | (((bt >> sh) & 15u) << 4));
+	}
+};
+
+}
diff --git a/rnamotif_b200/csrc/gpumotif.cu b/rnamotif_b200/csrc/gpumotif.cu
--- a/rnamotif_b200/csrc/gpumotif.cu
+++ b/rnamotif_b200/csrc/gpumotif.cu
@@ -116,6 +116,7 @@
 	bool use_split;
 	bool full;
 	int a_threads, a_blocks, b_threads, b_blocks;
+	bool a_packed;
 	size_t a_smem, b_smem;
 	uint32_t *d_wl;
 	size_t wl_cap;
@@ -188,8 +189,10 @@
 {
 	return full ? (search_kernel_t)gm_dfs_kernel<true> : (search_kernel_t)gm_dfs_kernel<false>;
 }
-static search_kernel_t pre_kernel(int pf)
-{
+static search_kernel_t pre_kernel(int pf, bool packed)
+{
+	if (packed)
+		return pf == 3 ? (search_kernel_t)gm_filter_packed_kernel<3> : (search_kernel_t)gm_filter_packed_kernel<2>;
 	return pf == 3 ? (search_kernel_t)gm_filter_kernel<3> : pf == 2 ? (search_kernel_t)gm_filter_kernel<2> :
 		pf == 1 ? (search_kernel_t)gm_filter_kernel<1> : (search_kernel_t)gm_filter_kernel<0>;
 }
@@ -847,13 +850,13 @@
 }
 
 
-static size_t smem_need(const gm_ctx *c, int threads, int tile, bool with_state = true)
+static size_t smem_need(const gm_ctx *c, int threads, int tile, bool with_state = true, bool seq_copies = true)
 {
 	const int Lb = (tile + 2 * c->par.halo + 31) & ~31;
 	const size_t stage = ((Lb >> 1) + 32 + 15) & ~15;
 	const size_t pb = (((size_t)2 * c->par.n_dups * 4 * (((Lb + 31) >> 5) + 4) * 4) + 15) & ~(size_t)15;
 	const size_t lit = c->par.lit_present ? (((size_t)2 * (((Lb + 31) >> 5) + 4) * 4) + 15) & ~(size_t)15 : 0;
-	const size_t buf_bytes = 2 * (size_t)Lb + pb + (GM_REC_CACHE + 2) * 8 + lit;
+	const size_t buf_bytes = (seq_copies ? 2 * (size_t)Lb : 0) + pb + (GM_REC_CACHE + 2) * 8 + lit;
 	const size_t warp_bytes = 16 + stage + (with_state ? 2 : 1) * buf_bytes + GM_QCAP * 2 +
 		(c->par.sieve ? ((6 * (size_t)(((Lb + 31) >> 5) + 4) * 4 + 15) & ~(size_t)15) : 0) +
 		(c->par.chain ? ((6 * (size_t)(((Lb + 31) >> 5) + 4) * 4 + 15) & ~(size_t)15) : 0);
@@ -973,23 +976,52 @@
 		const bool strong = c->par.pf_deep || c->par.chain || c->par.lit_present || est <= 0.5;
 		eligible = wtot <= 512 && ((c->par.sieve && strong) || (c->par.lit_present && c->full));
 	}
-	const int fused_tile0 = c->par.tile;
-	if (eligible && tile_arg <= 0 && c->par.sieve) {
-		for (int t2 = 1984; t2 >= 448; t2 = t2 == 1984 ? 960 : 448) {
-			if (smem_need(c, 256, t2, false) * 2 + 2048 <= smem_sm) {
-				tile = t2;
-				break;
+	const int fused_tile = c->par.tile;
+	c->use_split = false;
+	c->a_packed = c->par.sieve && c->par.chain > 0;
+	const search_kernel_t fk = pre_kernel(pre_pf(c->par), c->a_packed);
+	c->a_threads = 0;
+	if (eligible && c->a_packed) {
+		double best = 0;
+		int a_tile = tile;
+		if (cudaFuncSetAttribute(fk, cudaFuncAttributeMaxDynamicSharedMemorySize, GM_SMEM_OPTIN) == cudaSuccess) {
+			for (int n = 1; n <= 4; n++) {
+				const int t2 = tile_arg <= 0 ? 512 * n - 64 : tile;
+				for (int t = 64; t <= 256; t <<= 1) {
+					const size_t need = smem_need(c, t, t2, false, false);
+					int nb = 0;
+					if (need > smem_sm || cudaOccupancyMaxActiveBlocksPerMultiprocessor(&nb, fk, t, need) != cudaSuccess)
+						continue;
+					const double score = (double)nb * (t >> 5) * t2 / (t2 + 2.0 * c->par.halo);
+					if (nb > 0 && score > best * 1.001) {
+						best = score;
+						a_tile = t2;
+						c->a_threads = t;
+					}
+				}
+				if (tile_arg > 0)
+					break;
 			}
-			if (t2 == 448)
-				break;
-		}
+		}
+		cudaGetLastError();
+		tile = a_tile;
 		c->par.tile = tile;
-	}
-	const int fused_tile = fused_tile0;
-	c->use_split = false;
-	if (eligible) {
+	} else if (eligible) {
+		if (tile_arg <= 0 && c->par.sieve) {
+			for (int t2 = 1984; t2 >= 448; t2 = t2 == 1984 ? 960 : 448) {
+				if (smem_need(c, 256, t2, false) * 2 + 2048 <= smem_sm) {
+					tile = t2;
+					break;
+				}
+				if (t2 == 448)
+					break;
+			}
+			c->par.tile = tile;
+		}
 		c->a_threads = 256;
-		c->a_smem = smem_need(c, c->a_threads, tile, false);
+	}
+	if (c->a_threads > 0) {
+		c->a_smem = smem_need(c, c->a_threads, tile, false, !c->a_packed);
 		int best_w = 0;
 		c->b_threads = 0;
 		for (int t = 64; t <= 256; t <<= 1) {
@@ -1010,9 +1042,9 @@
 		cudaGetLastError();
 		int na = 0;
 		if (c->b_threads > 0 && c->a_smem <= smem_sm &&
-		    cudaFuncSetAttribute(pre_kernel(pre_pf(c->par)), cudaFuncAttributeMaxDynamicSharedMemorySize, GM_SMEM_OPTIN) == cudaSuccess &&
+		    cudaFuncSetAttribute(fk, cudaFuncAttributeMaxDynamicSharedMemorySize, GM_SMEM_OPTIN) == cudaSuccess &&
 		    cudaFuncSetAttribute(dfs_kernel(c->full), cudaFuncAttributeMaxDynamicSharedMemorySize, GM_SMEM_OPTIN) == cudaSuccess &&
-		    cudaOccupancyMaxActiveBlocksPerMultiprocessor(&na, pre_kernel(pre_pf(c->par)), c->a_threads, c->a_smem) == cudaSuccess &&
+		    cudaOccupancyMaxActiveBlocksPerMultiprocessor(&na, fk, c->a_threads, c->a_smem) == cudaSuccess &&
 		    na >= 1) {
 			c->a_blocks = na * c->n_sm;
 			c->use_split = true;
@@ -1022,8 +1054,9 @@
 	if (!c->use_split)
 		c->par.tile = fused_tile;
 	if (getenv("GPUMOTIF_DEBUG") != NULL && c->use_split)
-		fprintf(stderr, "gpumotif: split path, tile %d, sieve/prefilter %d x %d (%zu B), dfs %d x %d (%zu B)\n", c->par.tile,
-			c->a_blocks, c->a_threads, c->a_smem, c->b_blocks, c->b_threads, c->b_smem);
+		fprintf(stderr, "gpumotif: split path, tile %d, %s %d x %d (%d per SM, %d warps per SM, %zu B), dfs %d x %d (%zu B)\n",
+			c->par.tile, c->a_packed ? "packed sieve" : "sieve/prefilter", c->a_blocks, c->a_threads, c->a_blocks / c->n_sm,
+			c->a_blocks / c->n_sm * (c->a_threads >> 5), c->a_smem, c->b_blocks, c->b_threads, c->b_smem);
 	return 0;
 }
 
@@ -2241,7 +2274,7 @@
 				c->seg_ev.push_back(e);
 			}
 			CU(cudaEventRecord(c->seg_ev[2 * c->n_seg_ev], c->stream));
-			pre_kernel(pre_pf(c->par))<<<ablocks, c->a_threads, c->a_smem, c->stream>>>(A);
+			pre_kernel(pre_pf(c->par), c->a_packed)<<<ablocks, c->a_threads, c->a_smem, c->stream>>>(A);
 			CU(cudaGetLastError());
 			CU(cudaEventRecord(c->seg_ev[2 * c->n_seg_ev + 1], c->stream));
 			c->n_seg_ev++;
```

New measurement: 111.7, median of 6. 0.986x the previous value.
